# Crocodoctopus/zkstark

Measured on AMD Instinct MI355X. Metric: field-elements/s through LDE+Merkle+FRI (full STARK-101 prover), higher is better.
Workload: dtype u32 (mod 3*2^30+1) + SHA-256

## Files before the change

### zkstark_amd/csrc/host_sha.cpp

```cpp
#include "host_sha.hpp"

#include <atomic>

#if !defined(__HIP_DEVICE_COMPILE__)
#include <immintrin.h>
#include <stdlib.h>
#include <string.h>

namespace zk {
namespace {

#define ZK_SHA_TARGET __attribute__((target("sha,sse4.1,ssse3")))

alignas(16) const uint32_t K[64] = {
    0x428a2f98u, 0x71374491u, 0xb5c0fbcfu, 0xe9b5dba5u, 0x3956c25bu, 0x59f111f1u, 0x923f82a4u, 0xab1c5ed5u,
    0xd807aa98u, 0x12835b01u, 0x243185beu, 0x550c7dc3u, 0x72be5d74u, 0x80deb1feu, 0x9bdc06a7u, 0xc19bf174u,
    0xe49b69c1u, 0xefbe4786u, 0x0fc19dc6u, 0x240ca1ccu, 0x2de92c6fu, 0x4a7484aau, 0x5cb0a9dcu, 0x76f988dau,
    0x983e5152u, 0xa831c66du, 0xb00327c8u, 0xbf597fc7u, 0xc6e00bf3u, 0xd5a79147u, 0x06ca6351u, 0x14292967u,
    0x27b70a85u, 0x2e1b2138u, 0x4d2c6dfcu, 0x53380d13u, 0x650a7354u, 0x766a0abbu, 0x81c2c92eu, 0x92722c85u,
    0xa2bfe8a1u, 0xa81a664bu, 0xc24b8b70u, 0xc76c51a3u, 0xd192e819u, 0xd6990624u, 0xf40e3585u, 0x106aa070u,
    0x19a4c116u, 0x1e376c08u, 0x2748774cu, 0x34b0bcb5u, 0x391c0cb3u, 0x4ed8aa4au, 0x5b9cca4fu, 0x682e6ff3u,
    0x748f82eeu, 0x78a5636fu, 0x84c87814u, 0x8cc70208u, 0x90befffau, 0xa4506cebu, 0xbef9a3f7u, 0xc67178f2u};
const uint32_t IV[8] = {0x6a09e667u, 0xbb67ae85u, 0x3c6ef372u, 0xa54ff53au, 0x510e527fu, 0x9b05688cu, 0x1f83d9abu, 0x5be0cd19u};

alignas(16) uint32_t PADKW[64];
bool g_cpu_has_sha = false, g_cpu_has_x16 = false;
std::atomic<bool> g_have_sha{false}, g_have_x16{false};
std::atomic<bool> g_want_x16{true};

inline uint32_t rotr(uint32_t x, int n) { return (x >> n) | (x << (32 - n)); }

struct Init {
    Init() {
        __builtin_cpu_init();
        g_cpu_has_sha = __builtin_cpu_supports("sha") && __builtin_cpu_supports("sse4.1") && __builtin_cpu_supports("ssse3");
        g_cpu_has_x16 = g_cpu_has_sha && __builtin_cpu_supports("avx512f");
        g_have_sha = g_cpu_has_sha;
        g_have_x16 = g_cpu_has_x16;
        uint32_t w[64] = {0x80000000u};
        w[15] = 512u;
        for (int t = 16; t < 64; ++t) {
            uint32_t s0 = rotr(w[t - 15], 7) ^ rotr(w[t - 15], 18) ^ (w[t - 15] >> 3);
            uint32_t s1 = rotr(w[t - 2], 17) ^ rotr(w[t - 2], 19) ^ (w[t - 2] >> 10);
            w[t] = w[t - 16] + s0 + w[t - 7] + s1;
        }
        for (int t = 0; t < 64; ++t) PADKW[t] = K[t] + w[t];
    }
} g_init;

ZK_SHA_TARGET inline void load_state(const uint32_t st[8], __m128i& s0, __m128i& s1) {
    __m128i t = _mm_loadu_si128((const __m128i*)st);
    s1 = _mm_loadu_si128((const __m128i*)(st + 4));
    t = _mm_shuffle_epi32(t, 0xB1);
    s1 = _mm_shuffle_epi32(s1, 0x1B);
    s0 = _mm_alignr_epi8(t, s1, 8);
    s1 = _mm_blend_epi16(s1, t, 0xF0);
}
ZK_SHA_TARGET inline void store_state(uint32_t st[8], __m128i s0, __m128i s1) {
    __m128i t = _mm_shuffle_epi32(s0, 0x1B);
    s1 = _mm_shuffle_epi32(s1, 0xB1);
    s0 = _mm_blend_epi16(t, s1, 0xF0);
    s1 = _mm_alignr_epi8(s1, t, 8);
    _mm_storeu_si128((__m128i*)st, s0);
    _mm_storeu_si128((__m128i*)(st + 4), s1);
}

ZK_SHA_TARGET inline void rounds_msg(__m128i& s0, __m128i& s1, __m128i m[4]) {
    const __m128i a0 = s0, a1 = s1;
#pragma GCC unroll 16
    for (int g = 0; g < 16; ++g) {
        __m128i cur = m[g & 3];
        __m128i msg = _mm_add_epi32(cur, _mm_load_si128((const __m128i*)(K + 4 * g)));
        s1 = _mm_sha256rnds2_epu32(s1, s0, msg);
        if (g >= 3 && g <= 14) {
            __m128i t = _mm_alignr_epi8(cur, m[(g + 3) & 3], 4);
            m[(g + 1) & 3] = _mm_sha256msg2_epu32(_mm_add_epi32(m[(g + 1) & 3], t), cur);
        }
        msg = _mm_shuffle_epi32(msg, 0x0E);
        s0 = _mm_sha256rnds2_epu32(s0, s1, msg);
        if (g >= 1 && g <= 12) m[(g + 3) & 3] = _mm_sha256msg1_epu32(m[(g + 3) & 3], cur);
    }
    s0 = _mm_add_epi32(s0, a0);
    s1 = _mm_add_epi32(s1, a1);
}
ZK_SHA_TARGET inline void rounds_pad64(__m128i& s0, __m128i& s1) {
    const __m128i a0 = s0, a1 = s1;
#pragma GCC unroll 16
    for (int g = 0; g < 16; ++g) {
        __m128i msg = _mm_load_si128((const __m128i*)(PADKW + 4 * g));
        s1 = _mm_sha256rnds2_epu32(s1, s0, msg);
        msg = _mm_shuffle_epi32(msg, 0x0E);
        s0 = _mm_sha256rnds2_epu32(s0, s1, msg);
    }
    s0 = _mm_add_epi32(s0, a0);
    s1 = _mm_add_epi32(s1, a1);
}

ZK_SHA_TARGET void inner_ni(const uint32_t* l, const uint32_t* r, uint32_t* out) {
    __m128i s0, s1, m[4];
    load_state(IV, s0, s1);
    m[0] = _mm_loadu_si128((const __m128i*)l);
    m[1] = _mm_loadu_si128((const __m128i*)(l + 4));
    m[2] = _mm_loadu_si128((const __m128i*)r);
    m[3] = _mm_loadu_si128((const __m128i*)(r + 4));
    rounds_msg(s0, s1, m);
    rounds_pad64(s0, s1);
    store_state(out, s0, s1);
}
ZK_SHA_TARGET void inner_ni_x2(const uint32_t* in, uint32_t* out) {
    __m128i s0, s1, u0, u1, m[4], n[4];
    load_state(IV, s0, s1);
    u0 = s0; u1 = s1;
    const __m128i a0 = s0, a1 = s1;
    for (int i = 0; i < 4; ++i) {
        m[i] = _mm_loadu_si128((const __m128i*)(in + 4 * i));
        n[i] = _mm_loadu_si128((const __m128i*)(in + 16 + 4 * i));
    }
#pragma GCC unroll 16
    for (int g = 0; g < 16; ++g) {
        const __m128i k = _mm_load_si128((const __m128i*)(K + 4 * g));
        __m128i cm = m[g & 3], cn = n[g & 3];
        __m128i xm = _mm_add_epi32(cm, k), xn = _mm_add_epi32(cn, k);
        s1 = _mm_sha256rnds2_epu32(s1, s0, xm);
        u1 = _mm_sha256rnds2_epu32(u1, u0, xn);
        if (g >= 3 && g <= 14) {
            __m128i tm = _mm_alignr_epi8(cm, m[(g + 3) & 3], 4), tn = _mm_alignr_epi8(cn, n[(g + 3) & 3], 4);
            m[(g + 1) & 3] = _mm_sha256msg2_epu32(_mm_add_epi32(m[(g + 1) & 3], tm), cm);
            n[(g + 1) & 3] = _mm_sha256msg2_epu32(_mm_add_epi32(n[(g + 1) & 3], tn), cn);
        }
        xm = _mm_shuffle_epi32(xm, 0x0E);
        xn = _mm_shuffle_epi32(xn, 0x0E);
        s0 = _mm_sha256rnds2_epu32(s0, s1, xm);
        u0 = _mm_sha256rnds2_epu32(u0, u1, xn);
        if (g >= 1 && g <= 12) {
            m[(g + 3) & 3] = _mm_sha256msg1_epu32(m[(g + 3) & 3], cm);
            n[(g + 3) & 3] = _mm_sha256msg1_epu32(n[(g + 3) & 3], cn);
        }
    }
    s0 = _mm_add_epi32(s0, a0); s1 = _mm_add_epi32(s1, a1);
    u0 = _mm_add_epi32(u0, a0); u1 = _mm_add_epi32(u1, a1);
    const __m128i b0 = s0, b1 = s1, c0 = u0, c1 = u1;
#pragma GCC unroll 16
    for (int g = 0; g < 16; ++g) {
        __m128i msg = _mm_load_si128((const __m128i*)(PADKW + 4 * g));
        s1 = _mm_sha256rnds2_epu32(s1, s0, msg);
        u1 = _mm_sha256rnds2_epu32(u1, u0, msg);
        msg = _mm_shuffle_epi32(msg, 0x0E);
        s0 = _mm_sha256rnds2_epu32(s0, s1, msg);
        u0 = _mm_sha256rnds2_epu32(u0, u1, msg);
    }
    s0 = _mm_add_epi32(s0, b0); s1 = _mm_add_epi32(s1, b1);
    u0 = _mm_add_epi32(u0, c0); u1 = _mm_add_epi32(u1, c1);
    store_state(out, s0, s1);
    store_state(out + 8, u0, u1);
}
ZK_SHA_TARGET void compress_ni(uint32_t* st, const uint32_t* blk) {
    __m128i s0, s1, m[4];
    load_state(st, s0, s1);
    for (int i = 0; i < 4; ++i) m[i] = _mm_loadu_si128((const __m128i*)(blk + 4 * i));
    rounds_msg(s0, s1, m);
    store_state(st, s0, s1);
}
ZK_SHA_TARGET void blocks_ni(uint32_t* st, const uint8_t* data, size_t blocks) {
    const __m128i be = _mm_set_epi64x(0x0c0d0e0f08090a0bLL, 0x0405060700010203LL);
    __m128i s0, s1, m[4];
    load_state(st, s0, s1);
    for (; blocks; --blocks, data += 64) {
        for (int i = 0; i < 4; ++i) m[i] = _mm_shuffle_epi8(_mm_loadu_si128((const __m128i*)(data + 16 * i)), be);
        rounds_msg(s0, s1, m);
    }
    store_state(st, s0, s1);
}
ZK_SHA_TARGET void leaf_ni(uint32_t v, uint32_t* out) {
    __m128i s0, s1, m[4];
    load_state(IV, s0, s1);
    m[0] = _mm_set_epi32(0, 0, (int)0x80000000u, (int)v);
    m[1] = _mm_setzero_si128();
    m[2] = _mm_setzero_si128();
    m[3] = _mm_set_epi32(32, 0, 0, 0);
    rounds_msg(s0, s1, m);
    store_state(out, s0, s1);
}
#define ZK_X16_TARGET __attribute__((target("avx512f")))
#define ZK_ROR(x, n) _mm512_ror_epi32((x), (n))
#define ZK_XOR3(a, b, c) _mm512_ternarylogic_epi32((a), (b), (c), 0x96)

ZK_X16_TARGET inline void transpose16(__m512i r[16]) {
    __m512i t[16], u[16];
    for (int i = 0; i < 8; ++i) {
        t[2 * i] = _mm512_unpacklo_epi32(r[2 * i], r[2 * i + 1]);
        t[2 * i + 1] = _mm512_unpackhi_epi32(r[2 * i], r[2 * i + 1]);
    }
    for (int i = 0; i < 16; i += 4) {
        u[i] = _mm512_unpacklo_epi64(t[i], t[i + 2]);
        u[i + 1] = _mm512_unpackhi_epi64(t[i], t[i + 2]);
        u[i + 2] = _mm512_unpacklo_epi64(t[i + 1], t[i + 3]);
        u[i + 3] = _mm512_unpackhi_epi64(t[i + 1], t[i + 3]);
    }
    for (int k = 0; k < 4; ++k) {
        t[k] = _mm512_shuffle_i32x4(u[k], u[4 + k], 0x88);
        t[4 + k] = _mm512_shuffle_i32x4(u[k], u[4 + k], 0xdd);
        t[8 + k] = _mm512_shuffle_i32x4(u[8 + k], u[12 + k], 0x88);
        t[12 + k] = _mm512_shuffle_i32x4(u[8 + k], u[12 + k], 0xdd);
    }
    for (int k = 0; k < 4; ++k) {
        r[k] = _mm512_shuffle_i32x4(t[k], t[8 + k], 0x88);
        r[8 + k] = _mm512_shuffle_i32x4(t[k], t[8 + k], 0xdd);
        r[4 + k] = _mm512_shuffle_i32x4(t[4 + k], t[12 + k], 0x88);
        r[12 + k] = _mm512_shuffle_i32x4(t[4 + k], t[12 + k], 0xdd);
    }
}

template <bool MSG>
ZK_X16_TARGET inline void rounds_x16(__m512i st[8], __m512i w[16]) {
    __m512i a = st[0], b = st[1], c = st[2], d = st[3], e = st[4], f = st[5], g = st[6], h = st[7];
#pragma GCC unroll 64
    for (int t = 0; t < 64; ++t) {
        __m512i wk;
        if (MSG) {
            if (t >= 16) {
                const __m512i w15 = w[(t + 1) & 15], w2 = w[(t + 14) & 15];
                const __m512i s0 = ZK_XOR3(ZK_ROR(w15, 7), ZK_ROR(w15, 18), _mm512_srli_epi32(w15, 3));
                const __m512i s1 = ZK_XOR3(ZK_ROR(w2, 17), ZK_ROR(w2, 19), _mm512_srli_epi32(w2, 10));
                w[t & 15] = _mm512_add_epi32(_mm512_add_epi32(w[t & 15], s0), _mm512_add_epi32(w[(t + 9) & 15], s1));
            }
            wk = _mm512_add_epi32(w[t & 15], _mm512_set1_epi32((int)K[t]));
        } else {
            wk = _mm512_set1_epi32((int)PADKW[t]);
        }
        const __m512i S1 = ZK_XOR3(ZK_ROR(e, 6), ZK_ROR(e, 11), ZK_ROR(e, 25));
        const __m512i t1 = _mm512_add_epi32(_mm512_add_epi32(h, S1), _mm512_add_epi32(_mm512_ternarylogic_epi32(e, f, g, 0xCA), wk));
        const __m512i S0 = ZK_XOR3(ZK_ROR(a, 2), ZK_ROR(a, 13), ZK_ROR(a, 22));
        const __m512i t2 = _mm512_add_epi32(S0, _mm512_ternarylogic_epi32(a, b, c, 0xE8));
        h = g; g = f; f = e; e = _mm512_add_epi32(d, t1); d = c; c = b; b = a; a = _mm512_add_epi32(t1, t2);
    }
    st[0] = _mm512_add_epi32(st[0], a); st[1] = _mm512_add_epi32(st[1], b); st[2] = _mm512_add_epi32(st[2], c); st[3] = _mm512_add_epi32(st[3], d);
    st[4] = _mm512_add_epi32(st[4], e); st[5] = _mm512_add_epi32(st[5], f); st[6] = _mm512_add_epi32(st[6], g); st[7] = _mm512_add_epi32(st[7], h);
}
ZK_X16_TARGET inline void store_x16(const __m512i st[8], uint32_t* out) {
    __m512i r[16];
    for (int i = 0; i < 8; ++i) { r[i] = st[i]; r[8 + i] = _mm512_setzero_si512(); }
    transpose16(r);
    for (int n = 0; n < 16; ++n) _mm256_storeu_si256((__m256i*)(out + 8 * n), _mm512_castsi512_si256(r[n]));
}
ZK_X16_TARGET void inner_x16(const uint32_t* in, uint32_t* out) {
    __m512i w[16], st[8];
    for (int n = 0; n < 16; ++n) w[n] = _mm512_loadu_si512((const void*)(in + 16 * n));
    transpose16(w);
    for (int i = 0; i < 8; ++i) st[i] = _mm512_set1_epi32((int)IV[i]);
    rounds_x16<true>(st, w);
    rounds_x16<false>(st, w);
    store_x16(st, out);
}
ZK_X16_TARGET void leaves_x16(const uint32_t* vals, uint32_t* out) {
    __m512i w[16], st[8];
    w[0] = _mm512_loadu_si512((const void*)vals);
    w[1] = _mm512_set1_epi32((int)0x80000000u);
    for (int i = 2; i < 15; ++i) w[i] = _mm512_setzero_si512();
    w[15] = _mm512_set1_epi32(32);
    for (int i = 0; i < 8; ++i) st[i] = _mm512_set1_epi32((int)IV[i]);
    rounds_x16<true>(st, w);
    store_x16(st, out);
}

void inner_run(const uint32_t* child, uint32_t* out, size_t cnt) {
    size_t i = 0;
    if (g_have_x16)
        for (; i + 16 <= cnt; i += 16) inner_x16(child + 16 * i, out + 8 * i);
    for (; i + 2 <= cnt; i += 2) inner_ni_x2(child + 16 * i, out + 8 * i);
    for (; i < cnt; ++i) inner_ni(child + 16 * i, child + 16 * i + 8, out + 8 * i);
}

ZK_SHA_TARGET void reduce_ni(uint32_t* nodes, uint32_t depth) {
    for (uint32_t d = depth; d-- > 0;) {
        const size_t base = ((size_t)1 << d) - 1, child = ((size_t)2 << d) - 1, cnt = (size_t)1 << d;
        inner_run(nodes + 8 * child, nodes + 8 * base, cnt);
    }
}

ZK_SHA_TARGET void reduce_sub_ni(uint32_t* nodes, uint32_t depth, uint32_t top, size_t sub) {
    for (uint32_t d = depth; d-- > top;) {
        const size_t cnt = (size_t)1 << (d - top);
        const size_t base = ((size_t)1 << d) - 1 + sub * cnt, child = ((size_t)2 << d) - 1 + 2 * sub * cnt;
        inner_run(nodes + 8 * child, nodes + 8 * base, cnt);
    }
}

void compress_generic(uint32_t st[8], const uint32_t blk[16]) {
    uint32_t w[64];
    memcpy(w, blk, 64);
    for (int t = 16; t < 64; ++t) {
        uint32_t s0 = rotr(w[t - 15], 7) ^ rotr(w[t - 15], 18) ^ (w[t - 15] >> 3);
        uint32_t s1 = rotr(w[t - 2], 17) ^ rotr(w[t - 2], 19) ^ (w[t - 2] >> 10);
        w[t] = w[t - 16] + s0 + w[t - 7] + s1;
    }
    uint32_t a = st[0], b = st[1], c = st[2], d = st[3], e = st[4], f = st[5], g = st[6], h = st[7];
    for (int t = 0; t < 64; ++t) {
        uint32_t t1 = h + (rotr(e, 6) ^ rotr(e, 11) ^ rotr(e, 25)) + ((e & f) ^ (~e & g)) + K[t] + w[t];
        uint32_t t2 = (rotr(a, 2) ^ rotr(a, 13) ^ rotr(a, 22)) + ((a & b) ^ (a & c) ^ (b & c));
        h = g; g = f; f = e; e = d + t1; d = c; c = b; b = a; a = t1 + t2;
    }
    st[0] += a; st[1] += b; st[2] += c; st[3] += d; st[4] += e; st[5] += f; st[6] += g; st[7] += h;
}

}

bool host_sha_available() { return g_have_sha; }
void host_sha_use_extensions(bool on) {
    g_have_sha = on && g_cpu_has_sha;
    g_have_x16 = on && g_cpu_has_x16 && g_want_x16.load(std::memory_order_relaxed);
}
bool host_sha_wide_available() { return g_have_x16; }
void host_sha_use_wide(bool on) {
    g_want_x16 = on;
    g_have_x16 = on && g_have_sha.load(std::memory_order_relaxed) && g_cpu_has_x16;
}

void host_sha_compress(uint32_t state[8], const uint32_t block[16]) {
    if (g_have_sha) compress_ni(state, block);
    else compress_generic(state, block);
}

void host_sha_blocks(uint32_t state[8], const uint8_t* data, size_t blocks) {
    if (g_have_sha) { blocks_ni(state, data, blocks); return; }
    for (; blocks; --blocks, data += 64) {
        uint32_t w[16];
        for (int i = 0; i < 16; ++i)
            w[i] = ((uint32_t)data[4 * i] << 24) | ((uint32_t)data[4 * i + 1] << 16) | ((uint32_t)data[4 * i + 2] << 8) | data[4 * i + 3];
        compress_generic(state, w);
    }
}

void host_sha_leaf(uint32_t v, uint32_t out[8]) {
    if (g_have_sha) { leaf_ni(v, out); return; }
    uint32_t blk[16] = {v, 0x80000000u, 0, 0, 0, 0, 0, 0, 0, 0, 0, 0, 0, 0, 0, 32u};
    uint32_t st[8];
    memcpy(st, IV, 32);
    compress_generic(st, blk);
    memcpy(out, st, 32);
}

void host_sha_leaves(const uint32_t* vals, size_t n, uint32_t* out) {
    size_t i = 0;
    if (g_have_x16)
        for (; i + 16 <= n; i += 16) leaves_x16(vals + i, out + 8 * i);
    for (; i < n; ++i) host_sha_leaf(vals[i], out + 8 * i);
}

void host_sha_inner(const uint32_t left[8], const uint32_t right[8], uint32_t out[8]) {
    if (g_have_sha) { inner_ni(left, right, out); return; }
    uint32_t blk[16], st[8];
    memcpy(blk, left, 32);
    memcpy(blk + 8, right, 32);
    memcpy(st, IV, 32);
    compress_generic(st, blk);
    uint32_t pad[16] = {0x80000000u, 0, 0, 0, 0, 0, 0, 0, 0, 0, 0, 0, 0, 0, 0, 512u};
    compress_generic(st, pad);
    memcpy(out, st, 32);
}

void host_sha_inner_run(const uint32_t* children, uint32_t* out, size_t cnt) {
    if (g_have_sha) { inner_run(children, out, cnt); return; }
    for (size_t i = 0; i < cnt; ++i) host_sha_inner(children + 16 * i, children + 16 * i + 8, out + 8 * i);
}

void host_sha_reduce_sub(uint32_t* nodes, uint32_t depth, uint32_t top, size_t sub) {
    if (g_have_sha) { reduce_sub_ni(nodes, depth, top, sub); return; }
    for (uint32_t d = depth; d-- > top;) {
        const size_t cnt = (size_t)1 << (d - top);
        const size_t base = ((size_t)1 << d) - 1 + sub * cnt, child = ((size_t)2 << d) - 1 + 2 * sub * cnt;
        for (size_t i = 0; i < cnt; ++i)
            host_sha_inner(nodes + 8 * (child + 2 * i), nodes + 8 * (child + 2 * i + 1), nodes + 8 * (base + i));
    }
}

void host_sha_reduce(uint32_t* nodes, uint32_t depth) {
    if (g_have_sha) { reduce_ni(nodes, depth); return; }
    for (uint32_t d = depth; d-- > 0;) {
        const size_t base = ((size_t)1 << d) - 1, child = ((size_t)2 << d) - 1, cnt = (size_t)1 << d;
        for (size_t i = 0; i < cnt; ++i)
            host_sha_inner(nodes + 8 * (child + 2 * i), nodes + 8 * (child + 2 * i + 1), nodes + 8 * (base + i));
    }
}

}
#endif
```

### zkstark_amd/csrc/host_sha.hpp

```cpp
#pragma once
#include <stddef.h>
#include <stdint.h>

namespace zk {

bool host_sha_available();
void host_sha_use_extensions(bool on);
bool host_sha_wide_available();
void host_sha_use_wide(bool on);
void host_sha_compress(uint32_t state[8], const uint32_t block[16]);
void host_sha_blocks(uint32_t state[8], const uint8_t* data, size_t blocks);
void host_sha_leaf(uint32_t v, uint32_t out[8]);
void host_sha_leaves(const uint32_t* vals, size_t n, uint32_t* out);
void host_sha_inner(const uint32_t left[8], const uint32_t right[8], uint32_t out[8]);
void host_sha_inner_run(const uint32_t* children, uint32_t* out, size_t cnt);
void host_sha_reduce(uint32_t* nodes, uint32_t depth);
void host_sha_reduce_sub(uint32_t* nodes, uint32_t depth, uint32_t top, size_t sub);

}
```

### zkstark_amd/csrc/zkstark.hip

```cpp
#include <hip/hip_runtime.h>

#include <algorithm>
#include <chrono>
#include <cstdarg>
#include <cstdio>
#include <cstdlib>
#include <cstring>
#include <atomic>
#include <condition_variable>
#include <functional>
#include <mutex>
#include <new>
#include <thread>
#include <string>
#include <vector>

#include "../../include/zkstark_amd.h"
#include "field.hpp"
#include "kernels.hpp"
#include "sha256.hpp"
#include "transcript.hpp"
#include "host_sha.hpp"
#include "internal.hpp"
#include "pool.hpp"

using namespace zk;
using namespace zk::impl;

struct zk_ctx {
    int device = 0;
    uint32_t log_n = 0, log_b = 0, L = 0;
    size_t n = 0, N = 0, B = 0;
    uint32_t R = 0;
    hipStream_t stream = nullptr;
    zk_dom* dom = nullptr;
    uint32_t* d_trace = nullptr;
    uint32_t* d_coef = nullptr;
    uint32_t* d_layers = nullptr;
    std::vector<size_t> layer_off, layer_len;
    uint32_t* d_trees = nullptr;
    std::vector<size_t> tree_off;
    uint64_t* d_gather_off = nullptr;
    uint32_t* d_gather_out = nullptr;
    uint64_t* h_gather_off = nullptr;
    uint32_t* h_gather_out = nullptr;
    uint64_t* dm_gather_off = nullptr;
    uint32_t* dm_gather_out = nullptr;
    const uint32_t* host_nodes[40] = {};
    size_t host_node_cnt[40] = {};
    const uint32_t* host_vals[40] = {};
    std::vector<const uint32_t*> fetch_vals, fetch_nodes;
    std::vector<uint32_t> fetch_vdev;
    std::vector<uint64_t> fetch_ditems;
    std::vector<uint8_t> commit_buf;
    bool pending_top = false;
    uint32_t pending_tree = 0;
    size_t open_nv = 0, open_ndg = 0, open_vi = 0;
    bool open_pending = false;
    uint32_t* h_small = nullptr;
    uint32_t* h_mailbox = nullptr;
    uint32_t* d_mailbox = nullptr;
    uint32_t* d_counter = nullptr;
    bool counters_dirty = false;
    uint32_t mail_seq = 0;
    uint32_t tree_seq[40] = {};
    bool early = false, early_ok = false, gate_pending = false;
    uint32_t* h_gate = nullptr;
    uint32_t* d_gate = nullptr;
    uint32_t* h_dyn = nullptr;
    uint32_t* d_dyn = nullptr;
    uint32_t gate_seq = 0;
    uint32_t host_top = 0, host_tail = 0;
    Pool* pool = nullptr;
    uint32_t* h_stage = nullptr;
    uint32_t* d_stage = nullptr;
    size_t stage_words = 0, stage_used = 0;
    ScatterSeg* h_segs = nullptr;
    ScatterSeg* d_segs = nullptr;
    uint32_t n_segs = 0;
    double seg_words = 0;
    std::vector<uint32_t> tail_vals;
    uint32_t tail_log = 0;
    bool tail_have = false;
    double t_wait = 0, t_host_hash = 0, t_launch = 0;
    bool tail = false;
    uint32_t hinv_host = 0;
    ProofFormat fmt;
    Grinder* grinder = nullptr;
    uint64_t skipped_layers = 0, skipped_trees = 0;
    uint8_t tree_steps[40] = {};
    uint32_t* d_final = nullptr;
    std::vector<uint32_t> final_poly;
    int hash = 0;
    uint32_t cap_now = 0;
    uint8_t tree_cap[40] = {};
    std::vector<uint8_t> cap_digests[40];
    bool checks = false;
    uint32_t* d_check = nullptr;
    DevTable ones;
    size_t gather_cap = 0;
    size_t device_bytes = 0;
    double setup_ms = 0;
    bool have_trace = false, have_lde = false;
    uint32_t first = 0, last = 0;
    zk_transcript_info info{};
    Profiler prof;
    zk_kernel_stat kstat[K_COUNT] = {};
};

namespace {

template <typename T>
int dmalloc(zk_ctx* c, T** p, size_t bytes) {
    hipError_t e = hipMalloc((void**)p, bytes ? bytes : 4);
    if (e != hipSuccess) return fail(ZK_ERR_NOMEM, "hipMalloc(%zu) failed: %s", bytes, hipGetErrorString(e));
    c->device_bytes += bytes;
    return ZK_OK;
}

size_t layer_size(const zk_ctx* c, uint32_t layer) { return layer == 0 ? c->N : (c->N >> (layer - 1)); }
uint32_t layer_log(const zk_ctx* c, uint32_t layer) { return layer == 0 ? c->L : c->L - (layer - 1); }
uint32_t tree_log(const zk_ctx* c, uint32_t tree) { return layer_log(c, tree) - c->tree_steps[tree]; }
size_t tree_leaves(const zk_ctx* c, uint32_t tree) { return (size_t)1 << tree_log(c, tree); }

Profiler* prof_of(zk_ctx* c) { return c->prof.mask ? &c->prof : nullptr; }

void collect_kernel_stats(zk_ctx* c) {
    for (auto& r : c->prof.recs) {
        float ms = 0;
        (void)hipEventSynchronize(r.b);
        (void)hipEventElapsedTime(&ms, r.a, r.b);
        c->kstat[r.cls].launches += 1;
        c->kstat[r.cls].ms += ms;
        c->kstat[r.cls].bytes += r.bytes;
        c->kstat[r.cls].ops += r.ops;
        c->prof.pool.push_back(r.a);
        c->prof.pool.push_back(r.b);
    }
    c->prof.recs.clear();
}

int do_lde(zk_ctx* c) {
    int rc = dom_lde(c->dom, c->d_trace, c->d_coef, c->d_layers + c->layer_off[0], c->stream, prof_of(c));
    if (!rc) c->have_lde = true;
    return rc;
}

#ifndef ZK_HOST_SUB_LOG
#define ZK_HOST_SUB_LOG 8
#endif
static_assert(ZK_HOST_SUB_LOG >= 4 && ZK_HOST_SUB_LOG <= (int)kMaxHostLog, "host sub-tree size");
constexpr uint32_t host_sub_log() { return ZK_HOST_SUB_LOG; }
uint32_t top_of(const zk_ctx* c, uint32_t tree) {
    if (c->hash != 0 || !c->host_top) return 0;
    const uint32_t lg = tree_log(c, tree);
    return lg > c->host_top ? c->host_top : lg - 1;
}
uint32_t cap_of(const zk_ctx* c, uint32_t tree) { return c->cap_now ? cap_eff(c->cap_now, tree_log(c, tree)) : 0; }
uint32_t hand_of(const zk_ctx* c, uint32_t tree) {
    const uint32_t h = top_of(c, tree), ce = cap_of(c, tree);
    return h > ce ? h : ce;
}
MailArgs mail_of(zk_ctx* c, uint32_t tree, bool host, bool feed_tail = true, uint32_t steps = 0) {
    MailArgs m;
    c->tree_steps[tree] = (uint8_t)steps;
    if (c->counters_dirty) {
        (void)hipMemsetAsync(c->d_counter, 0, 64, c->stream);
        c->counters_dirty = false;
    }
    m.mailbox = c->d_mailbox;
    m.seq = ++c->mail_seq;
    c->tree_seq[tree] = m.seq;
    m.counter = c->d_counter;
    const uint32_t host_levels = host ? top_of(c, tree) : 0;
    c->tree_cap[tree] = (uint8_t)(host ? cap_of(c, tree) : 0);
    m.top = host ? hand_of(c, tree) : 0;
    if (feed_tail && c->fmt.fold == 1 && !c->fmt.coset && !c->fmt.stop && host_levels && c->host_tail && tree >= 1 && layer_log(c, tree) == c->host_tail + 1) {
        m.dump_src = c->d_layers + c->layer_off[tree];
        m.dump_log = c->host_tail + 1;
        m.vals_off = (uint32_t)kMailValsOff;
        c->tail_log = m.dump_log;
        c->tail_have = true;
    }
    return m;
}

int do_merkle(zk_ctx* c, uint32_t layer, bool host = false, bool feed_tail = true, uint32_t steps = 0) {
    HIPCHK(launch_merkle_build_coset(c->d_layers + c->layer_off[layer], layer_log(c, layer), steps, c->d_trees + c->tree_off[layer], c->stream,
                                     prof_of(c), mail_of(c, layer, host, feed_tail, steps), c->hash));
    return ZK_OK;
}

int do_compose_commit(zk_ctx* c, const uint32_t alpha_raw[3]) {
    ComposeArgs a;
    int rc = compose_args(c->dom, c->d_layers + c->layer_off[0], c->d_layers + c->layer_off[1], c->first, c->last, alpha_raw, a);
    if (rc) return rc;
    HIPCHK(launch_compose_merkle(a, c->d_trees + c->tree_off[1], c->stream, prof_of(c), mail_of(c, 1, true), c->hash));
    return ZK_OK;
}
int do_fold_commit(zk_ctx* c, uint32_t round, uint32_t beta_raw) {
    FoldArgs a;
    int rc = fold_args(c->dom, c->d_layers + c->layer_off[1 + round], c->d_layers + c->layer_off[2 + round], c->L - round, round, beta_raw, a);
    if (rc) return rc;
    HIPCHK(launch_fold_merkle(a, c->d_trees + c->tree_off[2 + round], c->stream, prof_of(c), mail_of(c, 2 + round, true), c->hash));
    return ZK_OK;
}

int wait_mail(zk_ctx* c, uint32_t seq) {
    double t0 = now_us();
    int rc = wait_flag(c->h_mailbox, seq, c->stream);
    c->t_wait += now_us() - t0;
    if (rc) c->counters_dirty = true;
    return rc;
}

int read_root(zk_ctx* c, uint32_t tree, uint8_t out[32]) {
    int rc = wait_mail(c, c->tree_seq[tree]);
    if (rc) return rc;
    digest_words_to_bytes(c->h_mailbox + kMailDigests, out);
    return ZK_OK;
}

uint32_t* stage_alloc(zk_ctx* c, size_t words) {
    if (c->stage_used + words > c->stage_words) return nullptr;
    uint32_t* p = c->h_stage + c->stage_used;
    c->stage_used += (words + 7) & ~(size_t)7;
    return p;
}
int stage_seg(zk_ctx* c, const uint32_t* src, size_t dst, size_t words, uint32_t kind) {
    if (c->n_segs >= 4 * 34) return fail(ZK_ERR_STATE, "scatter segment table full");
    c->h_segs[c->n_segs++] = ScatterSeg{(uint64_t)(src - c->h_stage), (uint64_t)dst, (uint32_t)words, kind};
    c->seg_words += (double)words;
    return ZK_OK;
}

int read_commit_cap(zk_ctx* c, uint32_t tree, uint32_t H, uint32_t ce, uint8_t root[32]) {
    const size_t cnt = (size_t)1 << H, first = ((size_t)1 << ce) - 1, ncap = (size_t)1 << ce;
    uint32_t* nodes = stage_alloc(c, (2 * cnt - 1) * 8);
    if (!nodes) return fail(ZK_ERR_STATE, "host staging buffer exhausted");
    int rc = wait_mail(c, c->tree_seq[tree]);
    if (rc) return rc;
    double t0 = now_us();
    memcpy(nodes + 8 * (cnt - 1), c->h_mailbox + kMailDigests, cnt * 32);
    if (H > ce) {
        if (c->pool) c->pool->run(ncap, 1, [&](size_t sub) { host_sha_reduce_sub(nodes, H, ce, sub); });
        else for (size_t sub = 0; sub < ncap; ++sub) host_sha_reduce_sub(nodes, H, ce, sub);
    }
    std::vector<uint8_t>& cd = c->cap_digests[tree];
    cd.resize(32 * ncap);
    for (size_t i = 0; i < ncap; ++i) digest_words_to_bytes(nodes + 8 * (first + i), cd.data() + 32 * i);
    memset(root, 0, 32);
    c->t_host_hash += now_us() - t0;
    if (c->tail_have && c->tail_log == layer_log(c, tree) && tree >= 1) {
        c->tail_vals.assign(c->h_mailbox + kMailValsOff, c->h_mailbox + kMailValsOff + ((size_t)1 << c->tail_log));
    }
    c->host_nodes[tree] = nodes;
    c->host_node_cnt[tree] = 2 * cnt - 1;
    return H > ce ? stage_seg(c, nodes + 8 * first, c->tree_off[tree] + 8 * first, (cnt - 1 - first) * 8, 0) : (int)ZK_OK;
}

int read_commit(zk_ctx* c, uint32_t tree, uint8_t root[32]) {
    const uint32_t H = hand_of(c, tree), ce = cap_of(c, tree);
    if (!H) return read_root(c, tree, root);
    if (ce) return read_commit_cap(c, tree, H, ce, root);
    const size_t cnt = (size_t)1 << H;
    uint32_t* nodes = stage_alloc(c, (2 * cnt - 1) * 8);
    if (!nodes) return fail(ZK_ERR_STATE, "host staging buffer exhausted");
    int rc = wait_mail(c, c->tree_seq[tree]);
    if (rc) return rc;
    double t0 = now_us();
    memcpy(nodes + 8 * (cnt - 1), c->h_mailbox + kMailDigests, cnt * 32);
    const uint32_t sub_log = host_sub_log();
    if (H > sub_log && c->pool) {
        const uint32_t top = H - sub_log;
        c->pool->run((size_t)1 << top, 1, [&](size_t sub) { host_sha_reduce_sub(nodes, H, top, sub); });
        host_sha_reduce(nodes, top);
    } else {
        host_sha_reduce(nodes, H);
    }
    digest_words_to_bytes(nodes, root);
    c->t_host_hash += now_us() - t0;
    if (c->tail_have && c->tail_log == layer_log(c, tree) && tree >= 1) {
        c->tail_vals.assign(c->h_mailbox + kMailValsOff, c->h_mailbox + kMailValsOff + ((size_t)1 << c->tail_log));
    }
    c->host_nodes[tree] = nodes;
    c->host_node_cnt[tree] = 2 * cnt - 1;
    return stage_seg(c, nodes, c->tree_off[tree], (cnt - 1) * 8, 0);
}

int host_fold_commit(zk_ctx* c, uint32_t round, uint32_t beta_raw, uint8_t root[32]) {
    const uint32_t log_out = c->L - round - 1;
    const size_t half = (size_t)1 << log_out;
    const double t_begin = now_us();
    uint32_t* vals = stage_alloc(c, half);
    uint32_t* nodes = stage_alloc(c, (2 * half - 1) * 8);
    if (!vals || !nodes) return fail(ZK_ERR_STATE, "host staging buffer exhausted");
    const zk_dom* d = c->dom;
    const uint32_t cc_m = to_mont(mulmod(beta_raw % P, d->fold_k[round]));
    const uint32_t step_m = to_mont(powmod(c->hinv_host, (uint64_t)1 << round));
    const uint32_t* in = c->tail_vals.data();
    uint32_t xinv_m = to_mont(1);
    for (size_t i = 0; i < half; ++i) {
        uint32_t u = in[i], v = in[i + half];
        vals[i] = add(mont_mul(add(u, v), d->inv2_mont), mont_mul(mont_mul(sub(u, v), xinv_m), cc_m));
        xinv_m = mont_mul(xinv_m, step_m);
    }
    host_sha_leaves(vals, half, nodes + 8 * (half - 1));
    host_sha_reduce(nodes, log_out);
    digest_words_to_bytes(nodes, root);
    c->tail_vals.assign(vals, vals + half);
    c->tail_log = log_out;
    c->t_host_hash += now_us() - t_begin;
    c->tree_steps[2 + round] = 0;
    c->tree_cap[2 + round] = (uint8_t)cap_of(c, 2 + round);
    if (const uint32_t ce = c->tree_cap[2 + round]) {
        std::vector<uint8_t>& cd = c->cap_digests[2 + round];
        cd.resize((size_t)32 << ce);
        for (size_t i = 0; i < ((size_t)1 << ce); ++i) digest_words_to_bytes(nodes + 8 * (((size_t)1 << ce) - 1 + i), cd.data() + 32 * i);
        memset(root, 0, 32);
    }
    c->host_vals[2 + round] = vals;
    c->host_nodes[2 + round] = nodes;
    c->host_node_cnt[2 + round] = 2 * half - 1;
    int rc = stage_seg(c, vals, c->layer_off[2 + round], half, 1);
    if (!rc) rc = stage_seg(c, nodes, c->tree_off[2 + round], (2 * half - 1) * 8, 0);
    return rc;
}

int fri_round_commit(zk_ctx* c, uint32_t round, uint32_t beta_raw, uint8_t root[32]) {
    if (c->tail_have && c->tail_log == c->L - round && c->L - round - 1 <= c->host_tail) return host_fold_commit(c, round, beta_raw, root);
    int rc = do_fold_commit(c, round, beta_raw);
    return rc ? rc : read_commit(c, 2 + round, root);
}
bool round_on_host(const zk_ctx* c, uint32_t round) {
    return c->hash == 0 && c->host_top && c->host_tail && c->L >= c->host_tail + 1 && c->L - round <= c->host_tail + 1;
}
bool can_gate(const zk_ctx* c, uint32_t round) { return c->fmt.fold == 1 && !c->fmt.coset && !c->fmt.stop && c->early && c->early_ok && !c->checks && round < c->R && !round_on_host(c, round); }
int enqueue_gated_fold(zk_ctx* c, uint32_t round) {
    FoldArgs a;
    int rc = fold_args(c->dom, c->d_layers + c->layer_off[1 + round], c->d_layers + c->layer_off[2 + round], c->L - round, round, 0u, a);
    if (rc) return rc;
    ++c->gate_seq;
    a.dyn = c->d_dyn + 16 * (c->gate_seq & 1u);
    HIPCHK(hipStreamWaitValue32(c->stream, c->d_gate, c->gate_seq, hipStreamWaitValueEq, 0xFFFFFFFFu));
    c->gate_pending = true;
    HIPCHK(launch_fold_merkle(a, c->d_trees + c->tree_off[2 + round], c->stream, prof_of(c), mail_of(c, 2 + round, true), c->hash));
    return ZK_OK;
}
void release_gate(zk_ctx* c, uint32_t c_mont) {
    c->h_dyn[16 * (c->gate_seq & 1u)] = c_mont;
    __atomic_store_n(c->h_gate, c->gate_seq, __ATOMIC_RELEASE);
    c->gate_pending = false;
}
void release_gated_fold(zk_ctx* c, uint32_t round, uint32_t beta_raw) {
    release_gate(c, to_mont(mulmod(beta_raw % P, c->dom->fold_k[round])));
}
struct GateGuard {
    zk_ctx* c;
    ~GateGuard() { if (c->gate_pending) release_gate(c, 0u); }
};

struct CapScope {
    zk_ctx* c;
    explicit CapScope(zk_ctx* ctx) : c(ctx) { c->cap_now = c->tail ? 0 : c->fmt.cap; }
    ~CapScope() { c->cap_now = 0; }
};

void begin_proof(zk_ctx* c) {
    c->stage_used = 0; c->n_segs = 0; c->seg_words = 0; c->tail_log = 0; c->tail_have = false;
    c->t_wait = c->t_host_hash = c->t_launch = 0;
    memset(c->host_nodes, 0, sizeof c->host_nodes);
    memset(c->host_node_cnt, 0, sizeof c->host_node_cnt);
    memset(c->host_vals, 0, sizeof c->host_vals);
}
int flush_host_parts(zk_ctx* c) {
    HIPCHK(launch_scatter(c->d_stage, c->d_segs, c->n_segs, c->seg_words, c->d_trees, c->d_layers, c->stream, prof_of(c)));
    c->n_segs = 0;
    c->pending_top = false;
    return ZK_OK;
}
int settle_pending(zk_ctx* c) { return c->pending_top ? flush_host_parts(c) : (int)ZK_OK; }
int last_layer_value(zk_ctx* c, uint32_t* out) {
    const uint32_t* v;
    if (c->tail_have && c->tail_log == c->log_b) v = c->tail_vals.data();
    else {
        HIPCHK(hipMemcpyAsync(c->h_small, c->d_layers + c->layer_off[1 + c->R], c->B * 4, hipMemcpyDeviceToHost, c->stream));
        HIPCHK(hipStreamSynchronize(c->stream));
        v = c->h_small;
    }
    for (size_t i = 1; i < c->B; ++i)
        if (v[i] != v[0]) return fail(ZK_ERR_CHECK, "last FRI layer is not constant (prover.rs:238): trace does not satisfy the constraints");
    *out = v[0];
    return ZK_OK;
}

int final_alloc(zk_ctx* c) {
    return c->d_final ? (int)ZK_OK : dmalloc(c, &c->d_final, (((size_t)1 << kFinalPolyMaxLog) + 1) * 4);
}
int final_poly_value(zk_ctx* c) {
    const uint32_t Rp = c->fmt.rounds();
    const size_t cnt = (size_t)1 << c->fmt.stop;
    int rc = final_alloc(c);
    if (rc) return rc;
    if ((rc = dom_final_poly(c->dom, c->d_layers + c->layer_off[1 + Rp], c->d_final, c->L - Rp, Rp, (uint32_t)cnt, c->stream, prof_of(c)))) return rc;
    HIPCHK(hipMemcpyAsync(c->h_small, c->d_final, (cnt + 1) * 4, hipMemcpyDeviceToHost, c->stream));
    HIPCHK(hipStreamSynchronize(c->stream));
    if (c->h_small[0])
        return fail(ZK_ERR_CHECK, "final FRI layer has degree >= 2^%u: trace does not satisfy the constraints (%u non-zero coefficients above; cf. prover.rs:238)", c->fmt.stop, c->h_small[0]);
    c->final_poly.assign(c->h_small + 1, c->h_small + 1 + cnt);
    return ZK_OK;
}

int do_compose(zk_ctx* c, const uint32_t alpha_raw[3]) {
    return dom_compose(c->dom, c->d_layers + c->layer_off[0], c->d_layers + c->layer_off[1], c->first, c->last,
                       alpha_raw, c->stream, prof_of(c));
}

int do_fold(zk_ctx* c, uint32_t round, uint32_t beta_raw) {
    return dom_fold(c->dom, c->d_layers + c->layer_off[1 + round], c->d_layers + c->layer_off[2 + round],
                    c->L - round, round, beta_raw, c->stream, prof_of(c));
}


int checks_alloc(zk_ctx* c) {
    if (c->d_check) return ZK_OK;
    int rc = dmalloc(c, &c->d_check, (c->N + 2) * 4);
    if (rc) return rc;
    return build_table(1, c->log_n, &c->ones);
}
int check_interpolant(zk_ctx* c) {
    const zk_dom* d = c->dom;
    CoefPrepArgs pa{};
    pa.log_n = d->log_n; pa.log_b = d->log_b;
    pa.tw = d->H.view(); pa.wtab = c->ones.view(); pa.ninv_mont = d->ninv_mont;
    pa.nd = d->plan.nd;
    for (uint32_t t = 0; t < d->plan.nd; ++t) pa.dig_bits[t] = d->plan.bits[t];
    HIPCHK(launch_coef_prepare(c->d_coef, c->d_check, pa, c->stream));
    int rc = run_dit(c->d_check, d->log_n, d->plan, d->H.view(), d->L, c->stream);
    if (rc) return rc;
    std::vector<uint32_t> got(c->n), want(c->n);
    HIPCHK(hipMemcpyAsync(got.data(), c->d_check, c->n * 4, hipMemcpyDeviceToHost, c->stream));
    HIPCHK(hipMemcpyAsync(want.data(), c->d_trace, c->n * 4, hipMemcpyDeviceToHost, c->stream));
    HIPCHK(hipStreamSynchronize(c->stream));
    for (size_t i = 0; i + 1 < c->n; ++i)
        if (got[i] != want[i])
            return fail(ZK_ERR_CHECK, "self-check prover.rs:64-66 failed: f(g^%zu) = %u, trace value %u", i, got[i], want[i]);
    return ZK_OK;
}
int check_degree(zk_ctx* c, uint32_t layer, uint32_t want_deg, const char* cite) {
    const uint32_t lg = layer_log(c, layer);
    const size_t m = (size_t)1 << lg;
    const uint32_t* src = c->d_layers + c->layer_off[layer];
    if (lg <= 10) {
        std::vector<uint32_t> v(m);
        if (c->tail_have && c->tail_log == lg && layer >= 2) v.assign(c->tail_vals.begin(), c->tail_vals.begin() + m);
        else {
            HIPCHK(hipMemcpyAsync(v.data(), src, m * 4, hipMemcpyDeviceToHost, c->stream));
            HIPCHK(hipStreamSynchronize(c->stream));
        }
        const uint32_t winv = invmod(root_of_unity(lg));
        for (size_t k = m; k-- > want_deg; ) {
            uint32_t acc = 0, step = powmod(winv, k), x = 1;
            for (size_t i = 0; i < m; ++i) { acc = add(acc, mulmod(v[i], x)); x = mulmod(x, step); }
            if (k > want_deg && acc != 0)
                return fail(ZK_ERR_CHECK, "self-check %s failed: layer %u has a non-zero coefficient of degree %zu > %u", cite, layer, k, want_deg);
            if (k == want_deg && acc == 0)
                return fail(ZK_ERR_CHECK, "self-check %s failed: layer %u has degree below %u", cite, layer, want_deg);
        }
        return ZK_OK;
    }
    const Plan pl = make_plan(lg);
    int rc = run_dif(src, c->d_check, lg, pl, c->dom->Hinv.view(), c->dom->L, 0, c->stream);
    if (rc) return rc;
    uint32_t* res = c->d_check + c->N;
    HIPCHK(hipMemsetAsync(res, 0, 8, c->stream));
    HIPCHK(launch_degree_check(c->d_check, lg, pl.nd, pl.bits, want_deg + 1, res, c->stream));
    uint32_t h[2];
    HIPCHK(hipMemcpyAsync(h, res, 8, hipMemcpyDeviceToHost, c->stream));
    HIPCHK(hipStreamSynchronize(c->stream));
    if (h[0]) return fail(ZK_ERR_CHECK, "self-check %s failed: layer %u has %u non-zero coefficients of degree > %u (a division left a remainder)", cite, layer, h[0], want_deg);
    if (!h[1]) return fail(ZK_ERR_CHECK, "self-check %s failed: layer %u has degree below %u", cite, layer, want_deg);
    return ZK_OK;
}

void open_begin(zk_ctx* c, size_t nvals) {
    c->fetch_vals.assign(nvals, nullptr); c->fetch_vdev.assign(nvals, 0); c->fetch_nodes.clear(); c->fetch_ditems.clear();
    c->open_nv = c->open_ndg = c->open_vi = 0;
}
void open_val(zk_ctx* c, uint32_t layer, size_t x) {
    if (c->host_vals[layer]) c->fetch_vals[c->open_vi++] = c->host_vals[layer] + x;
    else { c->fetch_vdev[c->open_vi++] = (uint32_t)c->open_nv; c->h_gather_off[c->open_nv++] = (uint64_t)c->layer_off[layer] + x; }
}
void open_path(zk_ctx* c, uint32_t tree, size_t m, size_t leaf) {
    const size_t stop_at = ((size_t)2 << c->tree_cap[tree]) - 2;
    for (size_t i = leaf + m - 1; i > stop_at; i = (i - 1) >> 1) {
        const size_t nd = (i & 1) ? i + 1 : i - 1;
        if (nd < c->host_node_cnt[tree]) c->fetch_nodes.push_back(c->host_nodes[tree] + 8 * nd);
        else { c->fetch_nodes.push_back(c->h_gather_out + 8 * c->open_ndg); ++c->open_ndg; c->fetch_ditems.push_back((uint64_t)c->tree_off[tree] + (uint64_t)nd * 8); }
    }
}
int open_launch(zk_ctx* c) {
    const size_t nv = c->open_nv, ndg = c->open_ndg;
    if (nv + ndg > c->gather_cap) return fail(ZK_ERR_STATE, "gather capacity exceeded");
    if (ndg) memcpy(c->h_gather_off + nv, c->fetch_ditems.data(), ndg * 8);
    for (size_t i = 0; i < c->fetch_vals.size(); ++i)
        if (!c->fetch_vals[i]) c->fetch_vals[i] = c->h_gather_out + 8 * ndg + c->fetch_vdev[i];
    c->open_pending = nv + ndg != 0;
    if (c->open_pending)
        HIPCHK(launch_fetch(c->d_layers, c->d_trees, c->dm_gather_off, (uint32_t)nv, (uint32_t)ndg, c->dm_gather_out, c->d_mailbox,
                            ++c->mail_seq, c->d_counter, c->stream, prof_of(c)));
    return ZK_OK;
}
int open_wait(zk_ctx* c) {
    if (!c->open_pending) return ZK_OK;
    c->open_pending = false;
    return wait_mail(c, c->mail_seq);
}

void commit_tree(zk_ctx* c, Channel& ch, uint32_t tree, const uint8_t root[32]) {
    if (c->tree_cap[tree]) { ch.commit_bytes(c->cap_digests[tree].data(), c->cap_digests[tree].size()); return; }
    ch.commit_hash(root);
    memcpy(c->info.roots[tree], root, 32);
}

int prove_fold_rounds(zk_ctx* c, Channel& ch) {
    const ProofFormat& f = c->fmt;
    const uint32_t R = f.rounds(), G = f.groups();
    uint8_t root[32];
    int rc;
    for (uint32_t j = 0; j < G; ++j) {
        const uint32_t r0 = f.round0(j), steps = f.steps(j), id = f.tree_id(j + 1);
        const uint32_t beta = c->info.beta_raw[r0] = ch.get_u32();
        if ((rc = dom_fold_multi(c->dom, c->d_layers + c->layer_off[1 + r0], c->d_layers + c->layer_off[id], c->L - r0, r0, steps, beta,
                                 c->stream, prof_of(c)))) return rc;
        const bool stopped = f.stop && j + 1 == G;
        if (!stopped && ((rc = do_merkle(c, id, true, false, f.slots_log(j + 1))) || (rc = read_commit(c, id, root)))) return rc;
        const size_t deg = c->n >> (r0 + steps);
        if (c->checks && (rc = check_degree(c, id, (uint32_t)deg - (deg ? 1 : 0), "prover.rs:228-251 (FRI layer degree)"))) return rc;
        if (!stopped) commit_tree(c, ch, id, root);
        for (uint32_t l = 2 + r0; l < id; ++l) { c->skipped_layers |= (uint64_t)1 << l; c->skipped_trees |= (uint64_t)1 << l; }
    }
    if (f.stop) {
        c->skipped_trees |= (uint64_t)1 << (1 + R);
        for (uint32_t l = 2 + R; l <= c->R + 1; ++l) { c->skipped_layers |= (uint64_t)1 << l; c->skipped_trees |= (uint64_t)1 << l; }
    }
    return ZK_OK;
}

struct HostLaps {
    const bool on;
    std::chrono::steady_clock::time_point t0 = std::chrono::steady_clock::now();
    void operator()(const char* what) {
        if (!on) return;
        auto t = std::chrono::steady_clock::now();
        fprintf(stderr, "[zk timing] %-28s %8.1f us\n", what, std::chrono::duration<double, std::micro>(t - t0).count());
        t0 = t;
    }
};

int prove_finish(zk_ctx* c, Channel& ch, HostLaps& lap) {
    const ProofFormat& f = c->fmt;
    const uint32_t Q = f.q;
    const size_t B = c->B, N = c->N;
    int rc;
    if (c->fmt.stop) {
        if ((rc = final_poly_value(c))) return rc;
        c->info.free_term = c->final_poly[0];
        std::vector<uint8_t>& cb = c->commit_buf;
        cb.resize(4 * c->final_poly.size());
        for (size_t k = 0; k < c->final_poly.size(); ++k)
            for (int i = 0; i < 4; ++i) cb[4 * k + i] = (uint8_t)(c->final_poly[k] >> (8 * i));
        ch.commit_bytes(cb.data(), cb.size());
    } else {
        uint32_t free_term = 0;
        if ((rc = last_layer_value(c, &free_term))) return rc;
        c->info.free_term = free_term;
        ch.commit_u32(free_term);
        c->final_poly.assign(1, free_term);
    }
    if (c->fmt.grind) {
        uint64_t w = 0;
        if ((rc = grind_channel(c->grinder, ch, c->fmt.grind, &w))) return rc;
        c->info.grind_bits = c->fmt.grind;
        c->info.grind_nonce = w;
        lap("grind");
    }
    uint32_t qraws[64];
    for (uint32_t k = 0; k < Q; ++k) qraws[k] = ch.get_u32();
    c->info.query_raw = qraws[0];

    size_t per_query = 0;
    f.for_each_tuple([&](size_t s, size_t, bool) { per_query += s; });
    open_begin(c, (size_t)Q * per_query);
    for (uint32_t k = 0; k < Q; ++k)
        f.for_each_opening((size_t)qraws[k] % (N - 2 * B), [&](uint32_t layer, uint32_t log_leaves, size_t leaf, uint32_t slots_log) {
            for (size_t u = 0; u < ((size_t)1 << slots_log); ++u) open_val(c, layer, leaf + (u << log_leaves));
            open_path(c, layer, (size_t)1 << log_leaves, leaf);
        });
    if ((rc = open_launch(c))) return rc;
    if ((rc = flush_host_parts(c))) return rc;
    lap("free term + fetch enqueue");
    if ((rc = open_wait(c))) return rc;
    lap("fetch wait");
    const uint32_t* const* vsrc = c->fetch_vals.data();
    const uint32_t* const* dsrc = c->fetch_nodes.data();
    std::vector<uint8_t>& buf = c->commit_buf;
    buf.resize(Channel::group_bytes((size_t)1 << f.steps(0), f.L(), false));
    auto tuple = [&](size_t s, size_t plen, bool one_leaf) {
        ch.commit_group(buf.data(), s, plen, [&](size_t t) { return *vsrc[t]; },
                        [&](size_t i, uint8_t* out) { digest_words_to_bytes(dsrc[i], out); }, one_leaf);
        vsrc += s; dsrc += (one_leaf ? 1 : s) * plen;
    };
    for (uint32_t q = 0; q < Q; ++q) f.for_each_tuple(tuple);
    lap("decommit host hashing");
    return ZK_OK;
}

int prove_resident(zk_ctx* c, Channel& ch) {
    if (!c->have_trace) return fail(ZK_ERR_STATE, "zk_prove_resident: no trace uploaded");
    static const bool timing = getenv("ZK_HOST_TIMING") != nullptr;
    HostLaps lap{timing};
    const uint32_t R = c->R;
    ch.data.reserve(ch.data.size() + c->fmt.data_len());
    CapScope cap_scope{c};
    c->skipped_layers = c->skipped_trees = 0;
    uint8_t root[32];
    int rc;
    memset(&c->info, 0, sizeof c->info);
    c->info.public_last = c->last;
    c->pending_top = false;
    begin_proof(c);
    GateGuard gate_guard{c};
    if ((rc = do_lde(c))) return rc;
    if (c->checks && ((rc = checks_alloc(c)) || (rc = check_interpolant(c)))) return rc;
    if ((rc = do_merkle(c, 0, true))) return rc;
    if ((rc = read_commit(c, 0, root))) return rc;
    commit_tree(c, ch, 0, root);
    uint32_t alpha[3];
    for (int i = 0; i < 3; ++i) alpha[i] = c->info.alpha_raw[i] = ch.get_u32();
    if (c->fmt.coset) {
        if ((rc = do_compose(c, alpha)) || (rc = do_merkle(c, 1, true, false, c->fmt.steps(0)))) return rc;
    } else if ((rc = do_compose_commit(c, alpha))) return rc;
    if (can_gate(c, 0) && (rc = enqueue_gated_fold(c, 0))) return rc;
    if ((rc = read_commit(c, 1, root))) return rc;
    if (c->checks && (rc = check_degree(c, 1, (uint32_t)c->n - 1, "prover.rs:148-159/:169 (exact divisions, deg cp = n - 1)"))) return rc;
    commit_tree(c, ch, 1, root);
    if (c->fmt.fold > 1 || c->fmt.coset || c->fmt.stop) {
        if ((rc = prove_fold_rounds(c, ch))) return rc;
    } else for (uint32_t r = 0; r < R; ++r) {
        uint32_t beta = c->info.beta_raw[r] = ch.get_u32();
        if (c->gate_pending) {
            release_gated_fold(c, r, beta);
            if (can_gate(c, r + 1) && (rc = enqueue_gated_fold(c, r + 1))) return rc;
            if ((rc = read_commit(c, 2 + r, root))) return rc;
        } else if (c->tail_have && c->tail_log == c->L - r && c->L - r - 1 <= c->host_tail) {
            if ((rc = host_fold_commit(c, r, beta, root))) return rc;
        } else {
            if ((rc = do_fold_commit(c, r, beta))) return rc;
            if (can_gate(c, r + 1) && (rc = enqueue_gated_fold(c, r + 1))) return rc;
            if ((rc = read_commit(c, 2 + r, root))) return rc;
        }
        if (c->checks && (rc = check_degree(c, 2 + r, (uint32_t)(c->n >> (r + 1)) - ((c->n >> (r + 1)) ? 1 : 0), "prover.rs:228-251 (FRI layer degree)"))) return rc;
        commit_tree(c, ch, 2 + r, root);
    }
    lap("lde .. last root");
    if (timing) fprintf(stderr, "[zk timing]   of which: waiting for the device %.1f us, host hashing (tops + tail) %.1f us\n", c->t_wait, c->t_host_hash);
    return prove_finish(c, ch, lap);
}

}

namespace zk {
namespace impl {
int tail_open_begin(zk_ctx* c, size_t x) {
    if (!c || !c->tail) return fail(ZK_ERR_INVALID, "tail_open_begin: not a tail context");
    HIPCHK(hipSetDevice(c->device));
    open_begin(c, 2 * (size_t)c->R);
    for (uint32_t i = 0; i < c->R; ++i) {
        const size_t len = c->N >> i, xi = x % len, nx = (xi + len / 2) % len;
        open_val(c, 1 + i, xi); open_path(c, 1 + i, len, xi);
        open_val(c, 1 + i, nx); open_path(c, 1 + i, len, nx);
    }
    return open_launch(c);
}
int tail_open_end(zk_ctx* c, uint32_t* vals_out, uint8_t* paths_out) {
    int rc = open_wait(c);
    if (rc) return rc;
    for (size_t i = 0; i < c->fetch_vals.size(); ++i) vals_out[i] = *c->fetch_vals[i];
    for (size_t i = 0; i < c->fetch_nodes.size(); ++i) digest_words_to_bytes(c->fetch_nodes[i], paths_out + 32 * i);
    return ZK_OK;
}
int merkle_nodes_to_host(int device, hipStream_t s, const uint32_t* d_heap, size_t first, size_t count, uint8_t* out) {
    if (!count) return ZK_OK;
    HIPCHK(hipSetDevice(device));
    HIPCHK(hipMemcpyAsync(out, d_heap + first * 8, count * 32, hipMemcpyDeviceToHost, s));
    HIPCHK(hipStreamSynchronize(s));
    for (size_t i = 0; i < count; ++i) {
        uint32_t w[8];
        memcpy(w, out + 32 * i, 32);
        digest_words_to_bytes(w, out + 32 * i);
    }
    return ZK_OK;
}
}
}

extern "C" {

const char* zk_last_error(void) { return last_error(); }
int zk_host_hash_mode(void) { return host_sha_wide_available() ? 2 : host_sha_available() ? 1 : 0; }
int zk_host_set_hash_mode(int mode) {
    if (mode < 0 || mode > 2) return fail(ZK_ERR_INVALID, "zk_host_set_hash_mode: mode %d out of range (0 portable, 1 SHA extensions, 2 + AVX-512)", mode);
    host_sha_use_extensions(mode >= 1);
    host_sha_use_wide(mode >= 2);
    return ZK_OK;
}

uint32_t zk_field_add(uint32_t a, uint32_t b) { return add(a % P, b % P); }
uint32_t zk_field_sub(uint32_t a, uint32_t b) { return sub(a % P, b % P); }
uint32_t zk_field_mul(uint32_t a, uint32_t b) { return mulmod(a % P, b % P); }
uint32_t zk_field_neg(uint32_t a) { return neg(a % P); }
uint32_t zk_field_inv(uint32_t a) { return invmod(a % P); }
uint32_t zk_field_pow(uint32_t a, uint32_t e) { return powmod(a, e); }
uint32_t zk_field_from_u32(uint32_t v) { return v % P; }
uint32_t zk_field_from_i32(int32_t v) {
    if (v < 0) return neg(uint32_t(-int64_t(v)) % P);
    return uint32_t(v) % P;
}
uint32_t zk_field_div(uint32_t a, uint32_t b) {
    if (b % P == 0) { fail(ZK_ERR_INVALID, "zk_field_div: division by zero (field.rs:165-177 panics)"); return 0; }
    return mulmod(a % P, invmod(b % P));
}
uint32_t zk_field_rem(uint32_t a, uint32_t rhs) {
    if (rhs == 0) { fail(ZK_ERR_INVALID, "zk_field_rem: remainder by zero (field.rs:89-94 panics)"); return 0; }
    return (a % P) % rhs;
}
uint32_t zk_field_generator(void) {
    static const uint32_t g = [] {
        uint32_t factors[32], nf = 0, p = P - 1;
        for (uint32_t it = 2; p != 1; ++it) {
            if (p % it == 0) factors[nf++] = it;
            while (p % it == 0) p /= it;
        }
        for (uint32_t x = 2; x < P; ++x) {
            bool primitive = true;
            for (uint32_t i = 0; i < nf && primitive; ++i) primitive = powmod(x, (P - 1) / factors[i]) != 1;
            if (primitive) return x;
        }
        return 0u;
    }();
    return g;
}
uint32_t zk_field_order(uint32_t a) {
    a %= P;
    if (a == 0) return 0;
    uint32_t ord = P - 1;
    if (powmod(a, ord / 3) == 1) ord /= 3;
    while (ord % 2 == 0 && powmod(a, ord / 2) == 1) ord /= 2;
    return ord;
}
uint32_t zk_field_root_of_unity(uint32_t log_order) { return log_order > 30 ? 0 : root_of_unity(log_order); }

static int ctx_make(int device, uint32_t log_n, uint32_t log_b, uint32_t shift, bool tail, zk_ctx** out);
static int ctx_team(zk_ctx* c) {
    const uint32_t sub_log = host_sub_log();
    const unsigned want = c->host_top > sub_log ? (1u << (c->host_top - sub_log)) - 1u : 0u;
    if (c->pool && c->pool->workers() == want) return ZK_OK;
    delete c->pool;
    c->pool = nullptr;
    if (!want) return ZK_OK;
    const double spin_us = 5000.0;
    c->pool = new (std::nothrow) Pool(want, spin_us);
    return c->pool ? (int)ZK_OK : fail(ZK_ERR_NOMEM, "out of host memory");
}

int zk_ctx_create(int device, uint32_t log_n, uint32_t log_b, zk_ctx** out) {
    if (!out) return fail(ZK_ERR_INVALID, "zk_ctx_create: out is null");
    *out = nullptr;
    if (int rc = check_proof_size("zk_ctx_create", log_n, log_b)) return rc;
    return ctx_make(device, log_n, log_b, GEN_W, false, out);
}

static int ctx_make(int device, uint32_t log_n, uint32_t log_b, uint32_t shift, bool tail, zk_ctx** out) {
    auto t0 = std::chrono::steady_clock::now();
    HIPCHK(hipSetDevice(device));
    zk_ctx* c = new (std::nothrow) zk_ctx();
    if (!c) return fail(ZK_ERR_NOMEM, "out of host memory");
    c->device = device;
    c->log_n = log_n; c->log_b = log_b; c->L = log_n + log_b;
    c->fmt.log_n = log_n; c->fmt.log_b = log_b;
    c->n = (size_t)1 << log_n; c->B = (size_t)1 << log_b; c->N = c->n << log_b;
    c->R = log_n;
    int rc = ZK_OK;
    auto bail = [&](int code) { zk_ctx_destroy(c); return code; };
#define HIPCHK_C(expr)                                                                        \
    do {                                                                                      \
        hipError_t _e = (expr);                                                               \
        if (_e != hipSuccess) {                                                               \
            zk_ctx_destroy(c);                                                                \
            return fail(ZK_ERR_HIP, "%s failed: %s (%s:%d)", #expr, hipGetErrorString(_e), __FILE__, __LINE__); \
        }                                                                                     \
    } while (0)
    HIPCHK_C(hipStreamCreateWithFlags(&c->stream, hipStreamNonBlocking));
    if ((rc = dom_make(device, log_n, log_b, shift, tail, c->stream, &c->dom))) return bail(rc);
    c->tail = tail;
    c->hinv_host = invmod(c->dom->h);
    c->device_bytes += c->dom->device_bytes;
    size_t off = 0;
    for (uint32_t l = 0; l <= c->R + 1; ++l) {
        c->layer_off.push_back(off);
        c->layer_len.push_back(layer_size(c, l));
        off += layer_size(c, l);
    }
    size_t layer_words = off;
    off = 0;
    for (uint32_t l = 0; l <= c->R + 1; ++l) {
        c->tree_off.push_back(off);
        off += (2 * layer_size(c, l) - 1) * 8;
    }
    size_t tree_words = off;
    if ((rc = dmalloc(c, &c->d_trace, c->n * 4))) return bail(rc);
    if ((rc = dmalloc(c, &c->d_coef, 2 * c->n * 4))) return bail(rc);
    if ((rc = dmalloc(c, &c->d_layers, layer_words * 4))) return bail(rc);
    if ((rc = dmalloc(c, &c->d_trees, tree_words * 4))) return bail(rc);
    c->gather_cap = (size_t)kMaxQueries * (4 + 2 * c->R) * (c->L + 1) + 64;
    if ((rc = dmalloc(c, &c->d_gather_off, c->gather_cap * 8))) return bail(rc);
    if ((rc = dmalloc(c, &c->d_gather_out, c->gather_cap * 32))) return bail(rc);
    HIPCHK_C(hipHostMalloc((void**)&c->h_gather_off, c->gather_cap * 8, hipHostMallocMapped | hipHostMallocCoherent));
    HIPCHK_C(hipHostMalloc((void**)&c->h_gather_out, c->gather_cap * 32, hipHostMallocMapped | hipHostMallocCoherent));
    HIPCHK_C(hipHostGetDevicePointer((void**)&c->dm_gather_off, c->h_gather_off, 0));
    HIPCHK_C(hipHostGetDevicePointer((void**)&c->dm_gather_out, c->h_gather_out, 0));
    HIPCHK_C(hipHostMalloc((void**)&c->h_small, 4096));
    const size_t mail_bytes = kMailWords * 4;
    if ((rc = dmalloc(c, &c->d_counter, 64))) return bail(rc);
    HIPCHK_C(hipMemsetAsync(c->d_counter, 0, 64, c->stream));
    HIPCHK_C(hipHostMalloc((void**)&c->h_mailbox, mail_bytes, hipHostMallocMapped | hipHostMallocCoherent));
    memset(c->h_mailbox, 0, mail_bytes);
    HIPCHK_C(hipHostGetDevicePointer((void**)&c->d_mailbox, c->h_mailbox, 0));
    HIPCHK_C(hipHostMalloc((void**)&c->h_gate, 64, hipHostMallocMapped | hipHostMallocCoherent));
    HIPCHK_C(hipHostMalloc((void**)&c->h_dyn, 2 * 16 * 4, hipHostMallocMapped | hipHostMallocCoherent));
    memset(c->h_gate, 0, 64);
    memset(c->h_dyn, 0, 2 * 16 * 4);
    HIPCHK_C(hipHostGetDevicePointer((void**)&c->d_gate, c->h_gate, 0));
    HIPCHK_C(hipHostGetDevicePointer((void**)&c->d_dyn, c->h_dyn, 0));
    {
        int can = 0;
        if (hipDeviceGetAttribute(&can, hipDeviceAttributeCanUseStreamWaitValue, device) != hipSuccess) { can = 0; (void)hipGetLastError(); }
        c->early_ok = can != 0 && !tail;
    }
    c->stage_words = (size_t)(c->R + 2) * ((size_t)16 << kMaxHostLog) + ((size_t)64 << kMaxHostLog);
    const size_t seg_bytes = 4 * 34 * sizeof(ScatterSeg);
    HIPCHK_C(hipHostMalloc((void**)&c->h_stage, c->stage_words * 4 + seg_bytes, hipHostMallocMapped | hipHostMallocCoherent));
    HIPCHK_C(hipHostGetDevicePointer((void**)&c->d_stage, c->h_stage, 0));
    c->h_segs = reinterpret_cast<ScatterSeg*>(c->h_stage + c->stage_words);
    c->d_segs = reinterpret_cast<ScatterSeg*>(c->d_stage + c->stage_words);
    if (host_sha_available()) {
        c->host_top = 8;
        c->host_tail = 9;
    }
    if (int prc = ctx_team(c)) { zk_ctx_destroy(c); return prc; }
#undef HIPCHK_C
    c->setup_ms = std::chrono::duration<double, std::milli>(std::chrono::steady_clock::now() - t0).count();
    *out = c;
    return ZK_OK;
}

#ifdef ZK_WG_TRACE
extern "C++" { namespace zk { void dump_wg_trace(); } }
#endif

int zk_ctx_destroy(zk_ctx* c) {
    if (!c) return ZK_OK;
    (void)hipSetDevice(c->device);
    if (c->stream) (void)hipStreamSynchronize(c->stream);
#ifdef ZK_WG_TRACE
    zk::dump_wg_trace();
#endif
    dom_free(c->dom);
    if (c->d_trace) (void)hipFree(c->d_trace);
    if (c->d_coef) (void)hipFree(c->d_coef);
    if (c->d_layers) (void)hipFree(c->d_layers);
    if (c->d_trees) (void)hipFree(c->d_trees);
    if (c->d_counter) (void)hipFree(c->d_counter);
    if (c->d_check) (void)hipFree(c->d_check);
    if (c->d_final) (void)hipFree(c->d_final);
    free_table(&c->ones);
    if (c->d_gather_off) (void)hipFree(c->d_gather_off);
    if (c->d_gather_out) (void)hipFree(c->d_gather_out);
    if (c->h_gather_off) (void)hipHostFree(c->h_gather_off);
    if (c->h_gather_out) (void)hipHostFree(c->h_gather_out);
    if (c->h_small) (void)hipHostFree(c->h_small);
    if (c->h_mailbox) (void)hipHostFree(c->h_mailbox);
    if (c->h_gate) (void)hipHostFree(c->h_gate);
    if (c->h_dyn) (void)hipHostFree(c->h_dyn);
    if (c->h_stage) (void)hipHostFree(c->h_stage);
    grinder_destroy(c->grinder);
    collect_kernel_stats(c);
    delete c->pool;
    for (hipEvent_t e : c->prof.pool) (void)hipEventDestroy(e);
    if (c->stream) (void)hipStreamDestroy(c->stream);
    delete c;
    return ZK_OK;
}

double zk_ctx_setup_ms(const zk_ctx* c) { return c ? c->setup_ms : 0.0; }
size_t zk_ctx_device_bytes(const zk_ctx* c) { return c ? c->device_bytes : 0; }
void* zk_ctx_stream(zk_ctx* c) {
    if (!c) return nullptr;
    if (c->pending_top && hipSetDevice(c->device) == hipSuccess) (void)settle_pending(c);
    return (void*)c->stream;
}
int zk_ctx_sync(zk_ctx* c) {
    if (!c) return fail(ZK_ERR_INVALID, "null context");
    HIPCHK(hipSetDevice(c->device));
    if (int rc = settle_pending(c)) return rc;
    HIPCHK(hipStreamSynchronize(c->stream));
    return ZK_OK;
}
int zk_ctx_set_early_launch(zk_ctx* c, int on) {
    if (!c) return fail(ZK_ERR_INVALID, "null context");
    c->early = on != 0;
    return ZK_OK;
}
int zk_ctx_get_early_launch(const zk_ctx* c) { return c && c->early && c->early_ok && c->fmt.fold == 1 && !c->fmt.coset && !c->fmt.stop ? 1 : 0; }
int zk_ctx_set_fold(zk_ctx* c, uint32_t fold_log) {
    if (!c) return fail(ZK_ERR_INVALID, "null context");
    if (c->tail) return fail(ZK_ERR_STATE, "zk_ctx_set_fold: FRI-tail context");
    if (fold_log < 1 || fold_log > kMaxFoldLog) return fail(ZK_ERR_INVALID, "zk_ctx_set_fold: need 1 <= fold_log <= %u (got %u)", kMaxFoldLog, fold_log);
    const ProofFormat widest{.log_n = c->log_n, .log_b = c->log_b, .fold = fold_log};
    size_t opened = 0;
    widest.for_each_tuple([&](size_t s, size_t, bool) { opened += s; });
    const size_t cap = (size_t)kMaxQueries * opened * (c->L + 1) + 64;
    if (cap > c->gather_cap) {
        HIPCHK(hipSetDevice(c->device));
        HIPCHK(hipStreamSynchronize(c->stream));
        uint64_t *d_off = nullptr, *h_off = nullptr, *dm_off = nullptr;
        uint32_t *d_out = nullptr, *h_out = nullptr, *dm_out = nullptr;
        hipError_t e = hipMalloc((void**)&d_off, cap * 8);
        if (e == hipSuccess) e = hipMalloc((void**)&d_out, cap * 32);
        if (e == hipSuccess) e = hipHostMalloc((void**)&h_off, cap * 8, hipHostMallocMapped | hipHostMallocCoherent);
        if (e == hipSuccess) e = hipHostMalloc((void**)&h_out, cap * 32, hipHostMallocMapped | hipHostMallocCoherent);
        if (e == hipSuccess) e = hipHostGetDevicePointer((void**)&dm_off, h_off, 0);
        if (e == hipSuccess) e = hipHostGetDevicePointer((void**)&dm_out, h_out, 0);
        if (e != hipSuccess) {
            if (d_off) (void)hipFree(d_off);
            if (d_out) (void)hipFree(d_out);
            if (h_off) (void)hipHostFree(h_off);
            if (h_out) (void)hipHostFree(h_out);
            return fail(ZK_ERR_NOMEM, "zk_ctx_set_fold: decommitment buffers: %s", hipGetErrorString(e));
        }
        (void)hipFree(c->d_gather_off); (void)hipFree(c->d_gather_out);
        (void)hipHostFree(c->h_gather_off); (void)hipHostFree(c->h_gather_out);
        c->d_gather_off = d_off; c->d_gather_out = d_out; c->h_gather_off = h_off; c->h_gather_out = h_out;
        c->dm_gather_off = dm_off; c->dm_gather_out = dm_out;
        c->device_bytes += (cap - c->gather_cap) * 40;
        c->gather_cap = cap;
    }
    c->fmt.fold = fold_log;
    return ZK_OK;
}
uint32_t zk_ctx_get_fold(const zk_ctx* c) { return c ? c->fmt.fold : 0; }
int zk_ctx_set_coset_leaves(zk_ctx* c, int on) {
    if (!c) return fail(ZK_ERR_INVALID, "null context");
    if (c->tail) return fail(ZK_ERR_STATE, "zk_ctx_set_coset_leaves: FRI-tail context");
    c->fmt.coset = on != 0;
    return ZK_OK;
}
int zk_ctx_get_coset_leaves(const zk_ctx* c) { return c && c->fmt.coset ? 1 : 0; }
int zk_ctx_set_fri_stop(zk_ctx* c, uint32_t stop_log) {
    if (!c) return fail(ZK_ERR_INVALID, "null context");
    if (c->tail) return fail(ZK_ERR_STATE, "zk_ctx_set_fri_stop: FRI-tail context");
    if (!stop_ok(c->log_n, c->log_b, stop_log))
        return fail(ZK_ERR_INVALID, "zk_ctx_set_fri_stop: need stop_log <= %u, stop_log <= log_n - 1 = %u and stop_log + log_blowup <= %u (got %u)",
                    kMaxStopLog, c->log_n - 1, kMaxStopLayerLog, stop_log);
    if (stop_log) {
        HIPCHK(hipSetDevice(c->device));
        if (int rc = final_alloc(c)) return rc;
    }
    c->fmt.stop = stop_log;
    return ZK_OK;
}
uint32_t zk_ctx_get_fri_stop(const zk_ctx* c) { return c ? c->fmt.stop : 0; }
int zk_ctx_final_poly(const zk_ctx* c, uint32_t* out, size_t cap, size_t* count) {
    if (!c || !count || (!out && cap)) return fail(ZK_ERR_INVALID, "zk_ctx_final_poly: null argument");
    if (c->final_poly.empty()) return fail(ZK_ERR_STATE, "zk_ctx_final_poly: no proof made yet");
    *count = c->final_poly.size();
    if (c->final_poly.size() > cap) return fail(ZK_ERR_BUFFER, "zk_ctx_final_poly: %zu coefficients, room for %zu", c->final_poly.size(), cap);
    memcpy(out, c->final_poly.data(), c->final_poly.size() * 4);
    return ZK_OK;
}
int zk_ctx_set_merkle_cap(zk_ctx* c, uint32_t cap_log) {
    if (!c) return fail(ZK_ERR_INVALID, "null context");
    if (c->tail) return fail(ZK_ERR_STATE, "zk_ctx_set_merkle_cap: FRI-tail context");
    if (cap_log > kMaxCapLog) return fail(ZK_ERR_INVALID, "zk_ctx_set_merkle_cap: need cap_log <= %u (got %u)", kMaxCapLog, cap_log);
    c->fmt.cap = cap_log;
    return ZK_OK;
}
uint32_t zk_ctx_get_merkle_cap(const zk_ctx* c) { return c ? c->fmt.cap : 0; }
uint32_t zk_ctx_merkle_cap_log(const zk_ctx* c, uint32_t tree) { return c && tree <= c->R + 1 ? c->tree_cap[tree] : 0; }
int zk_ctx_merkle_cap(const zk_ctx* c, uint32_t tree, uint8_t* out, size_t out_len) {
    if (!c || !out) return fail(ZK_ERR_INVALID, "zk_ctx_merkle_cap: null argument");
    if (tree > c->R + 1) return fail(ZK_ERR_INVALID, "zk_ctx_merkle_cap: tree %u out of range", tree);
    if (c->final_poly.empty()) return fail(ZK_ERR_STATE, "zk_ctx_merkle_cap: no proof made yet");
    if ((c->skipped_trees >> tree) & 1) return fail(ZK_ERR_STATE, "zk_ctx_merkle_cap: tree %u was not built by the last proof (fold_log %u, fri_stop %u)", tree, c->fmt.fold, c->fmt.stop);
    const uint32_t ce = c->tree_cap[tree];
    const uint8_t* src = ce ? c->cap_digests[tree].data() : c->info.roots[tree];
    if (((size_t)32 << ce) > out_len) return fail(ZK_ERR_BUFFER, "zk_ctx_merkle_cap: %zu bytes, room for %zu", (size_t)32 << ce, out_len);
    memcpy(out, src, (size_t)32 << ce);
    return ZK_OK;
}
int zk_ctx_set_queries(zk_ctx* c, uint32_t n_queries) {
    if (!c) return fail(ZK_ERR_INVALID, "null context");
    if (n_queries < 1 || n_queries > kMaxQueries) return fail(ZK_ERR_INVALID, "zk_ctx_set_queries: need 1 <= n_queries <= %u", kMaxQueries);
    c->fmt.q = n_queries;
    return ZK_OK;
}
int zk_ctx_set_grinding(zk_ctx* c, uint32_t grind_bits) {
    if (!c) return fail(ZK_ERR_INVALID, "null context");
    if (c->tail) return fail(ZK_ERR_STATE, "zk_ctx_set_grinding: FRI-tail context");
    if (grind_bits > kMaxGrindBits) return fail(ZK_ERR_INVALID, "zk_ctx_set_grinding: need grind_bits <= %u (got %u)", kMaxGrindBits, grind_bits);
    if (grind_bits > kGrindHostMaxBits && !c->grinder) {
        HIPCHK(hipSetDevice(c->device));
        if (int rc = grinder_create(c->device, c->stream, 1, &c->grinder)) return rc;
    }
    c->fmt.grind = grind_bits;
    return ZK_OK;
}

int zk_ctx_set_host_levels(zk_ctx* c, uint32_t top_log, uint32_t tail_log) {
    if (!c) return fail(ZK_ERR_INVALID, "null context");
    if (top_log > kMaxHostLog || tail_log > kMaxHostLog || (tail_log && !top_log))
        return fail(ZK_ERR_INVALID, "zk_ctx_set_host_levels: need top_log, tail_log <= %u, and top_log > 0 when tail_log > 0", kMaxHostLog);
    c->host_top = top_log;
    c->host_tail = tail_log;
    return ctx_team(c);
}
int zk_ctx_get_host_levels(const zk_ctx* c, uint32_t* top_log, uint32_t* tail_log) {
    if (!c || !top_log || !tail_log) return fail(ZK_ERR_INVALID, "zk_ctx_get_host_levels: null argument");
    *top_log = c->host_top;
    *tail_log = c->host_tail;
    return ZK_OK;
}
int zk_ctx_set_checks(zk_ctx* c, int on) {
    if (!c) return fail(ZK_ERR_INVALID, "null context");
    if (c->tail) return fail(ZK_ERR_STATE, "zk_ctx_set_checks: FRI-tail context");
    c->checks = on != 0;
    return ZK_OK;
}
static const char kNoBlake2s[] = "BLAKE2s (hash 2) is not built for this entry point yet";
int zk_ctx_set_hash(zk_ctx* c, int hash_kind) {
    if (!c) return fail(ZK_ERR_INVALID, "null context");
    if (hash_kind != ZK_HASH_SHA256 && hash_kind != ZK_HASH_FIELD && hash_kind != ZK_HASH_BLAKE2S)
        return fail(ZK_ERR_INVALID, "zk_ctx_set_hash: unknown hash %d", hash_kind);
    if (hash_kind == ZK_HASH_BLAKE2S && c->tail) return fail(ZK_ERR_INVALID, "zk_ctx_set_hash: %s", kNoBlake2s);
    c->hash = hash_kind;
    return ZK_OK;
}

int zk_ctx_set_profiling(zk_ctx* c, uint32_t class_mask) {
    if (!c) return fail(ZK_ERR_INVALID, "null context");
    c->prof.mask = class_mask & ((1u << K_COUNT) - 1u);
    return ZK_OK;
}

static int put_kernel_stats(zk_kernel_stat* out, size_t count, const zk_kernel_stat* src, const char* who) {
    if (!count) return ZK_OK;
    const uint32_t stride = out[0].struct_size;
    if (!abi_bytes(out, who)) return ZK_ERR_INVALID;
    for (size_t i = 0; i < count && i < (size_t)K_COUNT; ++i) {
        zk_kernel_stat* o = reinterpret_cast<zk_kernel_stat*>(reinterpret_cast<char*>(out) + i * stride);
        o->struct_size = stride;
        if (int rc = abi_put(o, src[i], who)) return rc;
    }
    return ZK_OK;
}

int zk_kernel_stats(zk_ctx* c, zk_kernel_stat* out, size_t count, int reset) {
    if (!c || (!out && count)) return fail(ZK_ERR_INVALID, "zk_kernel_stats: null argument");
    collect_kernel_stats(c);
    if (int rc = put_kernel_stats(out, count, c->kstat, "zk_kernel_stats")) return rc;
    if (reset) for (int i = 0; i < K_COUNT; ++i) c->kstat[i] = zk_kernel_stat{};
    return ZK_OK;
}

int zk_trace_fibsq(uint32_t a0, uint32_t a1, size_t count, uint32_t* out) {
    if (!out && count) return fail(ZK_ERR_INVALID, "zk_trace_fibsq: out is null");
    if (count > 0) out[0] = a0 % P;
    if (count > 1) out[1] = a1 % P;
    for (size_t i = 2; i < count; ++i)
        out[i] = add(mulmod(out[i - 2], out[i - 2]), mulmod(out[i - 1], out[i - 1]));
    return ZK_OK;
}

int zk_trace_upload(zk_ctx* c, const uint32_t* trace, size_t count) {
    if (!c || !trace) return fail(ZK_ERR_INVALID, "zk_trace_upload: null argument");
    if (count != c->n - 1) return fail(ZK_ERR_INVALID, "zk_trace_upload: expected n-1 = %zu values, got %zu", c->n - 1, count);
    for (size_t i = 0; i < count; ++i)
        if (trace[i] >= P) return fail(ZK_ERR_INVALID, "zk_trace_upload: trace[%zu] = %u is not a canonical residue", i, trace[i]);
    HIPCHK(hipSetDevice(c->device));
    HIPCHK(hipMemcpyAsync(c->d_trace, trace, count * 4, hipMemcpyHostToDevice, c->stream));
    HIPCHK(hipMemsetAsync(c->d_trace + count, 0, 4, c->stream));
    HIPCHK(hipStreamSynchronize(c->stream));
    c->first = trace[0];
    c->last = trace[count - 1];
    c->have_trace = true;
    c->have_lde = false;
    return ZK_OK;
}

int zk_lde(zk_ctx* c) {
    if (!c) return fail(ZK_ERR_INVALID, "null context");
    if (!c->have_trace) return fail(ZK_ERR_STATE, "zk_lde: no trace uploaded");
    HIPCHK(hipSetDevice(c->device));
    static const bool timing = getenv("ZK_HOST_TIMING") != nullptr;
    const double t0 = now_us();
    int rc = do_lde(c);
    if (timing) fprintf(stderr, "[zk timing] lde: enqueue of %u passes %.1f us\n", 2 * c->dom->plan.nd, now_us() - t0);
    return rc;
}

int zk_merkle_commit(zk_ctx* c, uint32_t layer, uint8_t root_out[32]) { return zk_merkle_commit_coset(c, layer, 0, root_out); }
int zk_merkle_commit_coset(zk_ctx* c, uint32_t layer, uint32_t steps, uint8_t root_out[32]) {
    if (!c || !root_out) return fail(ZK_ERR_INVALID, "zk_merkle_commit: null argument");
    if (layer > c->R + 1) return fail(ZK_ERR_INVALID, "zk_merkle_commit: layer %u out of range", layer);
    if (steps > kMaxFoldLog || (steps && layer_log(c, layer) <= steps))
        return fail(ZK_ERR_INVALID, "zk_merkle_commit_coset: need steps <= %u and at least two leaves (layer %u has 2^%u values, steps %u)", kMaxFoldLog, layer, layer_log(c, layer), steps);
    HIPCHK(hipSetDevice(c->device));
    static const bool timing = getenv("ZK_HOST_TIMING") != nullptr;
    const double t0 = now_us();
    c->skipped_trees &= ~((uint64_t)1 << layer);
    if (c->pending_top && c->pending_tree == layer) c->pending_top = false;
    int rc = settle_pending(c);
    if (rc) return rc;
    begin_proof(c);
    rc = do_merkle(c, layer, true, false, steps);
    const double t1 = now_us();
    if (!rc) rc = read_commit(c, layer, root_out);
    const double t2 = now_us();
    if (!rc && c->n_segs) { c->pending_top = true; c->pending_tree = layer; }
    if (timing)
        fprintf(stderr, "[zk timing] merkle_commit(layer %u): enqueue %.1f us, wait for the device %.1f us, host top %.1f us, scatter enqueue %.1f us\n",
                layer, t1 - t0, c->t_wait, c->t_host_hash, now_us() - t2);
    return rc;
}

int zk_compose(zk_ctx* c, const uint32_t alpha_raw[3]) {
    if (!c || !alpha_raw) return fail(ZK_ERR_INVALID, "zk_compose: null argument");
    if (!c->have_lde) return fail(ZK_ERR_STATE, "zk_compose: run zk_lde first");
    HIPCHK(hipSetDevice(c->device));
    return do_compose(c, alpha_raw);
}

int zk_fri_fold(zk_ctx* c, uint32_t round, uint32_t beta_raw) {
    if (!c) return fail(ZK_ERR_INVALID, "null context");
    if (round >= c->R) return fail(ZK_ERR_INVALID, "zk_fri_fold: round %u out of range (%u rounds)", round, c->R);
    HIPCHK(hipSetDevice(c->device));
    c->skipped_layers &= ~((uint64_t)1 << (2 + round));
    return do_fold(c, round, beta_raw);
}
int zk_fri_fold_multi(zk_ctx* c, uint32_t round, uint32_t steps, uint32_t beta_raw) {
    if (!c) return fail(ZK_ERR_INVALID, "null context");
    if (steps < 1 || steps > kMaxFoldLog) return fail(ZK_ERR_INVALID, "zk_fri_fold_multi: steps must be 1..%u (got %u)", kMaxFoldLog, steps);
    if (round >= c->R || round + steps > c->R) return fail(ZK_ERR_INVALID, "zk_fri_fold_multi: rounds %u..%u out of range (%u rounds)", round, round + steps, c->R);
    HIPCHK(hipSetDevice(c->device));
    c->skipped_layers &= ~((uint64_t)1 << (1 + round + steps));
    return dom_fold_multi(c->dom, c->d_layers + c->layer_off[1 + round], c->d_layers + c->layer_off[1 + round + steps], c->L - round, round, steps,
                          beta_raw, c->stream, prof_of(c));
}

int zk_fri_final_poly(zk_ctx* c, uint32_t layer, uint32_t bound, uint32_t* coef_out, uint32_t* high_nonzero) {
    if (!c || !coef_out || !high_nonzero) return fail(ZK_ERR_INVALID, "zk_fri_final_poly: null argument");
    if (layer < 1 || layer > c->R + 1) return fail(ZK_ERR_INVALID, "zk_fri_final_poly: layer %u out of range (FRI layers are 1..%u)", layer, c->R + 1);
    const uint32_t lg = layer_log(c, layer);
    if (lg > kFinalPolyMaxLog) return fail(ZK_ERR_INVALID, "zk_fri_final_poly: layer %u has 2^%u values, the limit is 2^%u", layer, lg, kFinalPolyMaxLog);
    if ((c->skipped_layers >> layer) & 1) return fail(ZK_ERR_STATE, "zk_fri_final_poly: layer %u was not materialised by the last proof", layer);
    HIPCHK(hipSetDevice(c->device));
    int rc = settle_pending(c);
    if (!rc) rc = final_alloc(c);
    if (!rc) rc = dom_final_poly(c->dom, c->d_layers + c->layer_off[layer], c->d_final, lg, layer - 1, bound, c->stream, prof_of(c));
    if (rc) return rc;
    HIPCHK(hipMemcpyAsync(high_nonzero, c->d_final, 4, hipMemcpyDeviceToHost, c->stream));
    HIPCHK(hipMemcpyAsync(coef_out, c->d_final + 1, ((size_t)4) << lg, hipMemcpyDeviceToHost, c->stream));
    HIPCHK(hipStreamSynchronize(c->stream));
    return ZK_OK;
}

int zk_layer_read(zk_ctx* c, uint32_t layer, size_t offset, size_t count, uint32_t* out) {
    if (!c || (!out && count)) return fail(ZK_ERR_INVALID, "zk_layer_read: null argument");
    if (layer > c->R + 1 || offset + count > layer_size(c, layer)) return fail(ZK_ERR_INVALID, "zk_layer_read: out of range");
    if ((c->skipped_layers >> layer) & 1) return fail(ZK_ERR_STATE, "zk_layer_read: layer %u was not materialised by the last proof (fold_log %u, fri_stop %u)", layer, c->fmt.fold, c->fmt.stop);
    HIPCHK(hipSetDevice(c->device));
    if (int prc = settle_pending(c)) return prc;
    HIPCHK(hipMemcpyAsync(out, c->d_layers + c->layer_off[layer] + offset, count * 4, hipMemcpyDeviceToHost, c->stream));
    HIPCHK(hipStreamSynchronize(c->stream));
    return ZK_OK;
}

int zk_layer_write(zk_ctx* c, uint32_t layer, size_t offset, size_t count, const uint32_t* in) {
    if (!c || (!in && count)) return fail(ZK_ERR_INVALID, "zk_layer_write: null argument");
    if (layer > c->R + 1 || offset + count > layer_size(c, layer)) return fail(ZK_ERR_INVALID, "zk_layer_write: out of range");
    for (size_t i = 0; i < count; ++i)
        if (in[i] >= P) return fail(ZK_ERR_INVALID, "zk_layer_write: value %zu is not a canonical residue", i);
    HIPCHK(hipSetDevice(c->device));
    HIPCHK(hipMemcpyAsync(c->d_layers + c->layer_off[layer] + offset, in, count * 4, hipMemcpyHostToDevice, c->stream));
    HIPCHK(hipStreamSynchronize(c->stream));
    if (layer == 0) c->have_lde = true;
    c->skipped_layers &= ~((uint64_t)1 << layer);
    return ZK_OK;
}

int zk_merkle_node(zk_ctx* c, uint32_t tree, size_t index, uint8_t out[32]) {
    if (!c || !out) return fail(ZK_ERR_INVALID, "zk_merkle_node: null argument");
    if (tree > c->R + 1 || index >= 2 * tree_leaves(c, tree) - 1) return fail(ZK_ERR_INVALID, "zk_merkle_node: out of range");
    if ((c->skipped_trees >> tree) & 1) return fail(ZK_ERR_STATE, "zk_merkle_node: tree %u was not built by the last proof (fold_log %u, fri_stop %u)", tree, c->fmt.fold, c->fmt.stop);
    if (index + 1 < ((size_t)1 << c->tree_cap[tree])) return fail(ZK_ERR_STATE, "zk_merkle_node: node %zu of tree %u lies above its Merkle cap (depth %u): the last proof did not build it", index, tree, c->tree_cap[tree]);
    HIPCHK(hipSetDevice(c->device));
    if (int prc = settle_pending(c)) return prc;
    HIPCHK(hipMemcpyAsync(c->h_small, c->d_trees + c->tree_off[tree] + index * 8, 32, hipMemcpyDeviceToHost, c->stream));
    HIPCHK(hipStreamSynchronize(c->stream));
    digest_words_to_bytes(c->h_small, out);
    return ZK_OK;
}

int zk_merkle_nodes(zk_ctx* c, uint32_t tree, size_t first, size_t count, uint8_t* out) {
    if (!c || (!out && count)) return fail(ZK_ERR_INVALID, "zk_merkle_nodes: null argument");
    if (tree > c->R + 1 || first > 2 * tree_leaves(c, tree) - 1 || count > 2 * tree_leaves(c, tree) - 1 - first)
        return fail(ZK_ERR_INVALID, "zk_merkle_nodes: out of range");
    if ((c->skipped_trees >> tree) & 1) return fail(ZK_ERR_STATE, "zk_merkle_nodes: tree %u was not built by the last proof (fold_log %u, fri_stop %u)", tree, c->fmt.fold, c->fmt.stop);
    if (count && first + 1 < ((size_t)1 << c->tree_cap[tree])) return fail(ZK_ERR_STATE, "zk_merkle_nodes: node %zu of tree %u lies above its Merkle cap (depth %u): the last proof did not build it", first, tree, c->tree_cap[tree]);
    HIPCHK(hipSetDevice(c->device));
    if (int prc = settle_pending(c)) return prc;
    return merkle_nodes_to_host(c->device, c->stream, c->d_trees + c->tree_off[tree], first, count, out);
}

int zk_merkle_path(zk_ctx* c, uint32_t tree, size_t leaf, uint8_t* out, size_t* path_len) {
    if (!c || !out) return fail(ZK_ERR_INVALID, "zk_merkle_path: null argument");
    if (tree > c->R + 1 || leaf >= tree_leaves(c, tree)) return fail(ZK_ERR_INVALID, "zk_merkle_path: out of range");
    if ((c->skipped_trees >> tree) & 1) return fail(ZK_ERR_STATE, "zk_merkle_path: tree %u was not built by the last proof (fold_log %u, fri_stop %u)", tree, c->fmt.fold, c->fmt.stop);
    if (c->tree_cap[tree]) return fail(ZK_ERR_STATE, "zk_merkle_path: tree %u was built down to its Merkle cap only (depth %u): a whole path does not exist", tree, c->tree_cap[tree]);
    HIPCHK(hipSetDevice(c->device));
    if (int prc = settle_pending(c)) return prc;
    std::vector<size_t> nodes;
    path_nodes(tree_leaves(c, tree), leaf, nodes);
    for (size_t i = 0; i < nodes.size(); ++i) c->h_gather_off[i] = (uint64_t)c->tree_off[tree] + (uint64_t)nodes[i] * 8;
    HIPCHK(hipMemcpyAsync(c->d_gather_off, c->h_gather_off, nodes.size() * 8, hipMemcpyHostToDevice, c->stream));
    HIPCHK(launch_gather(c->d_trees, c->d_gather_off, (uint32_t)nodes.size(), 8, c->d_gather_out, c->stream));
    HIPCHK(hipMemcpyAsync(c->h_gather_out, c->d_gather_out, nodes.size() * 32, hipMemcpyDeviceToHost, c->stream));
    HIPCHK(hipStreamSynchronize(c->stream));
    for (size_t i = 0; i < nodes.size(); ++i) digest_words_to_bytes(c->h_gather_out + 8 * i, out + 32 * i);
    if (path_len) *path_len = nodes.size();
    return ZK_OK;
}

int zk_prove_resident(zk_ctx* c, uint8_t* proof_out, size_t cap, size_t* proof_len, uint8_t state_out[32]) {
    if (!c || !proof_out || !state_out) return fail(ZK_ERR_INVALID, "zk_prove_resident: null argument");
    HIPCHK(hipSetDevice(c->device));
    Channel ch;
    int rc = prove_resident(c, ch);
    if (rc) return rc;
    const std::vector<uint8_t>& proof = ch.data;
    if (proof_len) *proof_len = proof.size();
    if (proof.size() > cap) return fail(ZK_ERR_BUFFER, "zk_prove: proof needs %zu bytes, buffer has %zu", proof.size(), cap);
    memcpy(proof_out, proof.data(), proof.size());
    memcpy(state_out, ch.state, 32);
    return ZK_OK;
}

int zk_prove_channel(zk_ctx* c, zk_channel* chan) {
    if (!c || !chan) return fail(ZK_ERR_INVALID, "zk_prove_channel: null argument");
    if (c->tail) return fail(ZK_ERR_STATE, "zk_prove_channel: FRI-tail context");
    HIPCHK(hipSetDevice(c->device));
    return prove_resident(c, chan->ch);
}

int zk_prove(zk_ctx* c, const uint32_t* trace, size_t count, uint8_t* proof_out, size_t cap, size_t* proof_len,
             uint8_t state_out[32]) {
    int rc = zk_trace_upload(c, trace, count);
    if (rc) return rc;
    return zk_prove_resident(c, proof_out, cap, proof_len, state_out);
}

int zk_prove_many(zk_ctx* const* ctxs, size_t count, uint8_t* proofs_out, size_t stride, size_t* lens_out, uint8_t* states_out) {
    if (!ctxs || !proofs_out || !lens_out || !states_out || count == 0 || count > 16)
        return fail(ZK_ERR_INVALID, "zk_prove_many: need 1..16 contexts and non-null outputs");
    for (size_t i = 0; i < count; ++i) {
        if (!ctxs[i]) return fail(ZK_ERR_INVALID, "zk_prove_many: context %zu is null", i);
        for (size_t j = 0; j < i; ++j)
            if (ctxs[j] == ctxs[i]) return fail(ZK_ERR_INVALID, "zk_prove_many: context %zu appears twice", i);
    }
    std::vector<int> rcs(count, ZK_OK);
    std::vector<std::string> errs(count);
    auto one = [&](size_t i) {
        rcs[i] = zk_prove_resident(ctxs[i], proofs_out + i * stride, stride, &lens_out[i], states_out + 32 * i);
        if (rcs[i]) errs[i] = last_error();
    };
    std::vector<std::thread> th;
    for (size_t i = 1; i < count; ++i) th.emplace_back(one, i);
    one(0);
    for (auto& t : th) t.join();
    for (size_t i = 0; i < count; ++i)
        if (rcs[i]) return fail(rcs[i], "zk_prove_many: context %zu: %s", i, errs[i].c_str());
    return ZK_OK;
}

int zk_last_transcript(const zk_ctx* c, zk_transcript_info* out) {
    if (!c || !out) return fail(ZK_ERR_INVALID, "zk_last_transcript: null argument");
    return abi_put(out, c->info, "zk_last_transcript");
}

static int verify_entry(const char* who, const uint8_t* proof, size_t len, const uint8_t* state, const ProofFormat& fmt, const uint32_t* public_last,
                        int hash_kind, int32_t* check_out, const char* replay_note, const char* reject_note) {
    if (hash_kind != ZK_HASH_SHA256 && hash_kind != ZK_HASH_FIELD && hash_kind != ZK_HASH_BLAKE2S) return fail(ZK_ERR_INVALID, "%s: unknown hash %d", who, hash_kind);
    if (fmt.fold < 1 || fmt.fold > kMaxFoldLog) return fail(ZK_ERR_INVALID, "%s: need 1 <= fold_log <= %u (got %u)", who, kMaxFoldLog, fmt.fold);
    if (fmt.cap > kMaxCapLog) return fail(ZK_ERR_INVALID, "%s: need cap_log <= %u (got %u)", who, kMaxCapLog, fmt.cap);
    int rc = state ? verify_transcript(proof, len, state, fmt) : 0;
    const bool in_replay = rc != 0;
    if (!rc) rc = verify_proof(proof, len, fmt, public_last, hash_kind);
    if (check_out) *check_out = rc;
    if (!rc) return ZK_OK;
    if (in_replay && replay_note) return fail(ZK_ERR_VERIFY, "transcript replay failed at check %d%s", rc, replay_note);
    return fail(ZK_ERR_VERIFY, "proof rejected at check %d%s", rc, reject_note);
}
static const char kProofRs[] = " (proof.rs:15-149)";

int zk_verify_ex(const uint8_t* proof, size_t len, uint32_t log_n, uint32_t log_b, uint32_t public_last, int hash_kind) {
    if (!proof) return fail(ZK_ERR_INVALID, "zk_verify: null proof");
    return verify_entry("zk_verify", proof, len, nullptr, ProofFormat{.log_n = log_n, .log_b = log_b}, &public_last, hash_kind, nullptr, nullptr, kProofRs);
}
int zk_verify(const uint8_t* proof, size_t len, uint32_t log_n, uint32_t log_b, uint32_t public_last) {
    return zk_verify_ex(proof, len, log_n, log_b, public_last, ZK_HASH_SHA256);
}
int zk_verify_queries(const uint8_t* proof, size_t len, const uint8_t* state, uint32_t log_n, uint32_t log_b, uint32_t public_last,
                      int hash_kind, uint32_t n_queries) {
    if (!proof) return fail(ZK_ERR_INVALID, "zk_verify_queries: null proof");
    return verify_entry("zk_verify_queries", proof, len, state, ProofFormat{.log_n = log_n, .log_b = log_b, .q = n_queries}, &public_last, hash_kind, nullptr, "", kProofRs);
}
int zk_verify_strict(const uint8_t* proof, size_t len, const uint8_t state[32], uint32_t log_n, uint32_t log_b, uint32_t public_last) {
    if (!proof || !state) return fail(ZK_ERR_INVALID, "zk_verify_strict: null argument");
    return verify_entry("zk_verify", proof, len, state, ProofFormat{.log_n = log_n, .log_b = log_b}, &public_last, ZK_HASH_SHA256, nullptr,
                        " (challenge not derived from the transcript, or final state mismatch)", kProofRs);
}
int zk_verify_grind(const uint8_t* proof, size_t len, const uint8_t* state, uint32_t log_n, uint32_t log_b, uint32_t public_last,
                    int hash_kind, uint32_t n_queries, uint32_t grind_bits, int32_t* check_out) {
    if (!proof || !check_out) return fail(ZK_ERR_INVALID, "zk_verify_check: null argument");
    return verify_entry("zk_verify_check", proof, len, state, ProofFormat{.log_n = log_n, .log_b = log_b, .q = n_queries, .grind = grind_bits}, &public_last, hash_kind,
                        check_out, nullptr, "");
}
int zk_verify_check(const uint8_t* proof, size_t len, const uint8_t* state, uint32_t log_n, uint32_t log_b, uint32_t public_last,
                    int hash_kind, uint32_t n_queries, int32_t* check_out) {
    if (hash_kind == ZK_HASH_BLAKE2S) return fail(ZK_ERR_INVALID, "zk_verify_check: BLAKE2s (hash 2) proofs are verified by zk_verify_stop");
    return zk_verify_grind(proof, len, state, log_n, log_b, public_last, hash_kind, n_queries, 0, check_out);
}
int zk_verify_fold(const uint8_t* proof, size_t len, const uint8_t* state, uint32_t log_n, uint32_t log_b, uint32_t public_last,
                   int hash_kind, uint32_t n_queries, uint32_t grind_bits, uint32_t fold_log, int32_t* check_out) {
    if (!proof || !check_out) return fail(ZK_ERR_INVALID, "zk_verify_fold: null argument");
    if (hash_kind == ZK_HASH_BLAKE2S) return fail(ZK_ERR_INVALID, "zk_verify_fold: BLAKE2s (hash 2) proofs are verified by zk_verify_stop");
    return verify_entry("zk_verify_fold", proof, len, state, ProofFormat{.log_n = log_n, .log_b = log_b, .q = n_queries, .grind = grind_bits, .fold = fold_log},
                        &public_last, hash_kind, check_out, nullptr, "");
}
int zk_verify_coset(const uint8_t* proof, size_t len, const uint8_t* state, uint32_t log_n, uint32_t log_b, uint32_t public_last,
                    int hash_kind, uint32_t n_queries, uint32_t grind_bits, uint32_t fold_log, int32_t* check_out) {
    if (!proof || !check_out) return fail(ZK_ERR_INVALID, "zk_verify_coset: null argument");
    return verify_entry("zk_verify_coset", proof, len, state,
                        ProofFormat{.log_n = log_n, .log_b = log_b, .q = n_queries, .grind = grind_bits, .fold = fold_log, .coset = true}, &public_last, hash_kind,
                        check_out, nullptr, "");
}
int zk_verify_stop(const uint8_t* proof, size_t len, const uint8_t* state, uint32_t log_n, uint32_t log_b, uint32_t public_last,
                   int hash_kind, uint32_t n_queries, uint32_t grind_bits, uint32_t fold_log, int coset_leaves, uint32_t stop_log, int32_t* check_out) {
    if (!proof || !check_out) return fail(ZK_ERR_INVALID, "zk_verify_stop: null argument");
    return verify_entry("zk_verify_stop", proof, len, state,
                        ProofFormat{.log_n = log_n, .log_b = log_b, .q = n_queries, .grind = grind_bits, .fold = fold_log, .coset = coset_leaves != 0, .stop = stop_log},
                        &public_last, hash_kind, check_out, nullptr, "");
}
int zk_verify_cap(const uint8_t* proof, size_t len, const uint8_t* state, uint32_t log_n, uint32_t log_b, uint32_t public_last,
                  int hash_kind, uint32_t n_queries, uint32_t grind_bits, uint32_t fold_log, int coset_leaves, uint32_t stop_log, uint32_t cap_log,
                  int32_t* check_out) {
    if (!proof || !check_out) return fail(ZK_ERR_INVALID, "zk_verify_cap: null argument");
    return verify_entry("zk_verify_cap", proof, len, state,
                        ProofFormat{.log_n = log_n, .log_b = log_b, .q = n_queries, .grind = grind_bits, .fold = fold_log, .coset = coset_leaves != 0, .stop = stop_log,
                                    .cap = cap_log},
                        &public_last, hash_kind, check_out, nullptr, "");
}
int zk_verify_shared(const uint8_t* proof, size_t len, const uint8_t* state, uint32_t log_n, uint32_t log_b, const uint32_t* public_last,
                     uint32_t log_batch, int hash_kind, uint32_t n_queries, uint32_t grind_bits, uint32_t fold_log, int coset_leaves, uint32_t stop_log,
                     uint32_t cap_log, int32_t* check_out) {
    if (!proof || !check_out || !public_last) return fail(ZK_ERR_INVALID, "zk_verify_shared: null argument");
    if (log_batch < 1 || log_batch > kMaxSharedLog) {
        *check_out = -1;
        return fail(ZK_ERR_INVALID, "zk_verify_shared: need 1 <= log_batch <= %u (got %u)", kMaxSharedLog, log_batch);
    }
    return verify_entry("zk_verify_shared", proof, len, state,
                        ProofFormat{.log_n = log_n, .log_b = log_b, .q = n_queries, .grind = grind_bits, .fold = fold_log, .coset = coset_leaves != 0, .stop = stop_log,
                                    .cap = cap_log, .lb = log_batch},
                        public_last, hash_kind, check_out, nullptr, "");
}
int zk_verify_shared_rows(const uint8_t* proof, size_t len, const uint8_t* state, uint32_t log_n, uint32_t log_b, const uint32_t* public_last,
                          uint32_t log_batch, int hash_kind, uint32_t n_queries, uint32_t grind_bits, uint32_t fold_log, int coset_leaves, uint32_t stop_log,
                          uint32_t cap_log, int row_leaves, int32_t* check_out) {
    if (!row_leaves)
        return zk_verify_shared(proof, len, state, log_n, log_b, public_last, log_batch, hash_kind, n_queries, grind_bits, fold_log, coset_leaves, stop_log, cap_log,
                                check_out);
    if (!proof || !check_out || !public_last) return fail(ZK_ERR_INVALID, "zk_verify_shared_rows: null argument");
    if (log_batch < 1 || log_batch > kMaxSharedLog) {
        *check_out = -1;
        return fail(ZK_ERR_INVALID, "zk_verify_shared_rows: row leaves need 1 <= log_batch <= %u (got %u)", kMaxSharedLog, log_batch);
    }
    if (hash_kind == ZK_HASH_BLAKE2S) {
        *check_out = -1;
        return fail(ZK_ERR_INVALID, "zk_verify_shared_rows: no BLAKE2s (hash 2) row leaves: no prover makes such a proof");
    }
    return verify_entry("zk_verify_shared_rows", proof, len, state,
                        ProofFormat{.log_n = log_n, .log_b = log_b, .q = n_queries, .grind = grind_bits, .fold = fold_log, .coset = coset_leaves != 0, .stop = stop_log,
                                    .cap = cap_log, .lb = log_batch, .rows = true},
                        public_last, hash_kind, check_out, nullptr, "");
}

size_t zk_proof_size(size_t data_len) { return 48 + data_len; }
size_t zk_proof_data_len_fold(uint32_t log_n, uint32_t log_b, uint32_t n_queries, uint32_t grind_bits, uint32_t fold_log) {
    if (fold_log < 1 || fold_log > kMaxFoldLog) return 0;
    return ProofFormat{.log_n = log_n, .log_b = log_b, .q = n_queries, .grind = grind_bits, .fold = fold_log}.data_len();
}
size_t zk_proof_data_len_coset(uint32_t log_n, uint32_t log_b, uint32_t n_queries, uint32_t grind_bits, uint32_t fold_log) {
    if (fold_log < 1 || fold_log > kMaxFoldLog) return 0;
    return ProofFormat{.log_n = log_n, .log_b = log_b, .q = n_queries, .grind = grind_bits, .fold = fold_log, .coset = true}.data_len();
}
size_t zk_proof_data_len_stop(uint32_t log_n, uint32_t log_b, uint32_t n_queries, uint32_t grind_bits, uint32_t fold_log, int coset_leaves, uint32_t stop_log) {
    if (fold_log < 1 || fold_log > kMaxFoldLog || !stop_ok(log_n, log_b, stop_log)) return 0;
    return ProofFormat{.log_n = log_n, .log_b = log_b, .q = n_queries, .grind = grind_bits, .fold = fold_log, .coset = coset_leaves != 0, .stop = stop_log}.data_len();
}
size_t zk_proof_data_len_cap(uint32_t log_n, uint32_t log_b, uint32_t n_queries, uint32_t grind_bits, uint32_t fold_log, int coset_leaves, uint32_t stop_log,
                             uint32_t cap_log) {
    if (fold_log < 1 || fold_log > kMaxFoldLog || !stop_ok(log_n, log_b, stop_log) || cap_log > kMaxCapLog) return 0;
    return ProofFormat{.log_n = log_n, .log_b = log_b, .q = n_queries, .grind = grind_bits, .fold = fold_log, .coset = coset_leaves != 0, .stop = stop_log, .cap = cap_log}
        .data_len();
}
size_t zk_proof_data_len_shared(uint32_t log_n, uint32_t log_b, uint32_t n_queries, uint32_t grind_bits, uint32_t fold_log, int coset_leaves, uint32_t stop_log,
                                uint32_t cap_log, uint32_t log_batch) {
    if (fold_log < 1 || fold_log > kMaxFoldLog || !stop_ok(log_n, log_b, stop_log) || cap_log > kMaxCapLog || log_batch > kMaxSharedLog) return 0;
    return ProofFormat{.log_n = log_n, .log_b = log_b, .q = n_queries, .grind = grind_bits, .fold = fold_log, .coset = coset_leaves != 0, .stop = stop_log, .cap = cap_log,
                       .lb = log_batch}
        .data_len();
}
size_t zk_proof_data_len_shared_rows(uint32_t log_n, uint32_t log_b, uint32_t n_queries, uint32_t grind_bits, uint32_t fold_log, int coset_leaves, uint32_t stop_log,
                                     uint32_t cap_log, uint32_t log_batch, int row_leaves) {
    if (fold_log < 1 || fold_log > kMaxFoldLog || !stop_ok(log_n, log_b, stop_log) || cap_log > kMaxCapLog || log_batch > kMaxSharedLog) return 0;
    if (row_leaves && log_batch < 1) return 0;
    return ProofFormat{.log_n = log_n, .log_b = log_b, .q = n_queries, .grind = grind_bits, .fold = fold_log, .coset = coset_leaves != 0, .stop = stop_log, .cap = cap_log,
                       .lb = log_batch, .rows = row_leaves != 0}
        .data_len();
}
size_t zk_proof_data_len_grind(uint32_t log_n, uint32_t log_b, uint32_t n_queries, uint32_t grind_bits) {
    return zk_proof_data_len_fold(log_n, log_b, n_queries, grind_bits, 1);
}
size_t zk_proof_data_len_queries(uint32_t log_n, uint32_t log_b, uint32_t n_queries) { return zk_proof_data_len_fold(log_n, log_b, n_queries, 0, 1); }
size_t zk_proof_data_len(uint32_t log_n, uint32_t log_b) { return zk_proof_data_len_fold(log_n, log_b, 1, 0, 1); }

int zk_compute_root_from_path_ex(uint32_t element, size_t index, const uint8_t* path, size_t path_len, uint8_t out[32], int hash_kind) {
    if ((!path && path_len) || !out || path_len > 62 || hash_kind < ZK_HASH_SHA256 || hash_kind > ZK_HASH_BLAKE2S)
        return fail(ZK_ERR_INVALID, "zk_compute_root_from_path: bad argument");
    compute_root_from_path(element, index, path, path_len, out, hash_kind);
    return ZK_OK;
}
int zk_compute_root_from_coset(const uint32_t* values, uint32_t s, size_t leaf, const uint8_t* path, size_t path_len, uint8_t out[32], int hash_kind) {
    if (!values || (!path && path_len) || !out || path_len > 62 || hash_kind < ZK_HASH_SHA256 || hash_kind > ZK_HASH_BLAKE2S || (s != 1 && s != 2 && s != 4 && s != 8))
        return fail(ZK_ERR_INVALID, "zk_compute_root_from_coset: bad argument");
    compute_root_from_coset(values, s, leaf, path, path_len, out, hash_kind);
    return ZK_OK;
}
int zk_compute_root_from_path(uint32_t element, size_t index, const uint8_t* path, size_t path_len, uint8_t out[32]) {
    return zk_compute_root_from_path_ex(element, index, path, path_len, out, ZK_HASH_SHA256);
}


int zk_tail_create(int device, uint32_t log_n_tail, uint32_t log_b, uint32_t shift, zk_ctx** out) {
    if (!out) return fail(ZK_ERR_INVALID, "zk_tail_create: out is null");
    *out = nullptr;
    if (log_n_tail < 1 || log_b < 1 || log_b > 5 || log_n_tail + log_b > 30)
        return fail(ZK_ERR_INVALID, "zk_tail_create: bad sizes (%u, %u)", log_n_tail, log_b);
    return ctx_make(device, log_n_tail, log_b, shift, true, out);
}

int zk_tail_run(zk_ctx* c, const uint32_t* d_layer0, void* src_stream, zk_channel* chan, int hash_kind,
                uint32_t* betas_out, uint8_t* roots_out, uint32_t* free_term_out) {
    if (hash_kind == ZK_HASH_BLAKE2S) return fail(ZK_ERR_INVALID, "zk_tail_run: %s", kNoBlake2s);
    if (!c || !c->tail || !d_layer0 || !chan || !betas_out || !roots_out || !free_term_out)
        return fail(ZK_ERR_INVALID, "zk_tail_run: bad argument");
    if (hash_kind != ZK_HASH_SHA256 && hash_kind != ZK_HASH_FIELD) return fail(ZK_ERR_INVALID, "zk_tail_run: unknown hash %d", hash_kind);
    HIPCHK(hipSetDevice(c->device));
    c->hash = hash_kind;
    HIPCHK(hipStreamSynchronize((hipStream_t)src_stream));
    HIPCHK(hipMemcpyAsync(c->d_layers + c->layer_off[1], d_layer0, c->N * 4, hipMemcpyDeviceToDevice, c->stream));
    Channel& ch = chan->ch;
    uint8_t root[32];
    int rc;
    begin_proof(c);
    if ((rc = do_merkle(c, 1, true))) return rc;
    if ((rc = read_commit(c, 1, root))) return rc;
    ch.commit_hash(root);
    memcpy(roots_out, root, 32);
    for (uint32_t r = 0; r < c->R; ++r) {
        uint32_t beta = betas_out[r] = ch.get_u32();
        if ((rc = fri_round_commit(c, r, beta, root))) return rc;
        ch.commit_hash(root);
        memcpy(roots_out + 32 * (r + 1), root, 32);
    }
    if ((rc = last_layer_value(c, free_term_out))) return rc;
    return flush_host_parts(c);
}

int zk_tail_open(zk_ctx* c, size_t x, uint32_t* vals_out, uint8_t* paths_out) {
    if (!c || !c->tail || !vals_out || !paths_out) return fail(ZK_ERR_INVALID, "zk_tail_open: bad argument");
    int rc = tail_open_begin(c, x);
    return rc ? rc : tail_open_end(c, vals_out, paths_out);
}
int zk_channel_new(zk_channel** out) {
    if (!out) return fail(ZK_ERR_INVALID, "null argument");
    *out = new (std::nothrow) zk_channel();
    return *out ? ZK_OK : fail(ZK_ERR_NOMEM, "out of host memory");
}
int zk_channel_free(zk_channel* ch) { delete ch; return ZK_OK; }
int zk_channel_import(zk_channel* ch, const uint8_t state[32], const uint8_t* data, size_t n) {
    if (!ch || !state || (!data && n)) return fail(ZK_ERR_INVALID, "null argument");
    memcpy(ch->ch.state, state, 32);
    ch->ch.data.assign(data, data + n);
    return ZK_OK;
}
int zk_channel_commit(zk_channel* ch, const uint8_t* bytes, size_t n) {
    if (!ch || (!bytes && n)) return fail(ZK_ERR_INVALID, "null argument");
    ch->ch.commit_bytes(bytes, n);
    return ZK_OK;
}
int zk_channel_get_u32(zk_channel* ch, uint32_t* out) {
    if (!ch || !out) return fail(ZK_ERR_INVALID, "null argument");
    *out = ch->ch.get_u32();
    return ZK_OK;
}
int zk_channel_state(const zk_channel* ch, uint8_t out[32]) {
    if (!ch || !out) return fail(ZK_ERR_INVALID, "null argument");
    memcpy(out, ch->ch.state, 32);
    return ZK_OK;
}
size_t zk_channel_data_len(const zk_channel* ch) { return ch ? ch->ch.data.size() : 0; }
int zk_channel_data(const zk_channel* ch, uint8_t* out, size_t cap) {
    if (!ch || !out) return fail(ZK_ERR_INVALID, "null argument");
    if (ch->ch.data.size() > cap) return fail(ZK_ERR_BUFFER, "buffer too small");
    memcpy(out, ch->ch.data.data(), ch->ch.data.size());
    return ZK_OK;
}

static Profiler g_dev_prof;
static zk_kernel_stat g_dev_kstat[K_COUNT] = {};
static Profiler* dev_prof() { return g_dev_prof.mask ? &g_dev_prof : nullptr; }

int zk_dev_set_profiling(uint32_t class_mask) {
    g_dev_prof.mask = class_mask & ((1u << K_COUNT) - 1u);
    return ZK_OK;
}
int zk_dev_kernel_stats(zk_kernel_stat* out, size_t count, int reset) {
    if (!out && count) return fail(ZK_ERR_INVALID, "zk_dev_kernel_stats: null argument");
    for (auto& r : g_dev_prof.recs) {
        float ms = 0;
        (void)hipEventSynchronize(r.b);
        (void)hipEventElapsedTime(&ms, r.a, r.b);
        g_dev_kstat[r.cls].launches += 1; g_dev_kstat[r.cls].ms += ms; g_dev_kstat[r.cls].bytes += r.bytes; g_dev_kstat[r.cls].ops += r.ops;
        g_dev_prof.pool.push_back(r.a); g_dev_prof.pool.push_back(r.b);
    }
    g_dev_prof.recs.clear();
    if (int rc = put_kernel_stats(out, count, g_dev_kstat, "zk_dev_kernel_stats")) return rc;
    if (reset) for (int i = 0; i < K_COUNT; ++i) g_dev_kstat[i] = zk_kernel_stat{};
    return ZK_OK;
}

int zk_dom_create(int device, uint32_t log_n, uint32_t log_b, uint32_t shift, int fold_only, zk_dom** out) {
    if (!out) return fail(ZK_ERR_INVALID, "zk_dom_create: out is null");
    return dom_make(device, log_n, log_b, shift, fold_only != 0, nullptr, out);
}
int zk_dom_destroy(zk_dom* d) {
    if (d) { (void)hipSetDevice(d->device); dom_free(d); }
    return ZK_OK;
}
int zk_dev_lde(const zk_dom* d, const uint32_t* d_trace, uint32_t* d_coef, uint32_t* d_out, void* stream) {
    if (!d || !d_trace || !d_coef || !d_out) return fail(ZK_ERR_INVALID, "zk_dev_lde: null argument");
    if (!d->d_inv_xm1) return fail(ZK_ERR_STATE, "zk_dev_lde: fold-only domain");
    HIPCHK(hipSetDevice(d->device));
    return dom_lde(d, d_trace, d_coef, d_out, (hipStream_t)stream, dev_prof());
}
int zk_dev_compose(const zk_dom* d, const uint32_t* d_f, uint32_t* d_cp, uint32_t first, uint32_t last,
                   const uint32_t alpha_raw[3], void* stream) {
    if (!d || !d_f || !d_cp || !alpha_raw) return fail(ZK_ERR_INVALID, "zk_dev_compose: null argument");
    if (!d->d_inv_xm1) return fail(ZK_ERR_STATE, "zk_dev_compose: fold-only domain");
    HIPCHK(hipSetDevice(d->device));
    return dom_compose(d, d_f, d_cp, first, last, alpha_raw, (hipStream_t)stream, dev_prof());
}
int zk_dev_fri_fold(const zk_dom* d, const uint32_t* d_in, uint32_t* d_out, uint32_t log_m, uint32_t round,
                    uint32_t beta_raw, void* stream) {
    if (!d || !d_in || !d_out) return fail(ZK_ERR_INVALID, "zk_dev_fri_fold: null argument");
    HIPCHK(hipSetDevice(d->device));
    return dom_fold(d, d_in, d_out, log_m, round, beta_raw, (hipStream_t)stream, dev_prof());
}
int zk_dev_fri_fold_multi(const zk_dom* d, const uint32_t* d_in, uint32_t* d_out, uint32_t log_m, uint32_t round, uint32_t steps,
                          uint32_t beta_raw, void* stream) {
    if (!d || !d_in || !d_out) return fail(ZK_ERR_INVALID, "zk_dev_fri_fold_multi: null argument");
    if (steps < 1 || steps > kMaxFoldLog) return fail(ZK_ERR_INVALID, "zk_dev_fri_fold_multi: steps must be 1..%u (got %u)", kMaxFoldLog, steps);
    if (round + steps > d->log_n || log_m + round != d->L)
        return fail(ZK_ERR_INVALID, "zk_dev_fri_fold_multi: layer 2^%u, rounds %u..%u do not fit a domain of %u rounds", log_m, round, round + steps, d->log_n);
    HIPCHK(hipSetDevice(d->device));
    return dom_fold_multi(d, d_in, d_out, log_m, round, steps, beta_raw, (hipStream_t)stream, dev_prof());
}
int zk_dev_fri_fold_multi_batch(const zk_dom* d, const uint32_t* d_in, uint32_t* d_out, uint32_t log_m, uint32_t round, uint32_t steps,
                                const uint32_t* d_beta_raw, uint32_t* d_work, uint32_t batch, void* stream) {
    if (!d || !d_in || !d_out || !d_beta_raw || !d_work) return fail(ZK_ERR_INVALID, "zk_dev_fri_fold_multi_batch: null argument");
    if (steps < 1 || steps > kMaxFoldLog) return fail(ZK_ERR_INVALID, "zk_dev_fri_fold_multi_batch: steps must be 1..%u (got %u)", kMaxFoldLog, steps);
    if (round + steps > d->log_n || log_m + round != d->L)
        return fail(ZK_ERR_INVALID, "zk_dev_fri_fold_multi_batch: layer 2^%u, rounds %u..%u do not fit a domain of %u rounds", log_m, round, round + steps, d->log_n);
    if (batch < 1 || ((uint64_t)batch << log_m) > ((uint64_t)1 << 32))
        return fail(ZK_ERR_INVALID, "zk_dev_fri_fold_multi_batch: need batch >= 1 and batch * 2^log_m <= 2^32 (got %u, log_m %u)", batch, log_m);
    HIPCHK(hipSetDevice(d->device));
    return dom_fold_multi_batch(d, d_in, d_out, log_m, round, steps, d_beta_raw, 1, d_work, batch, (hipStream_t)stream, dev_prof());
}
int zk_dev_trace_fibsq_batch(const uint32_t* d_a0, const uint32_t* d_a1, uint32_t batch, uint32_t count, uint32_t* d_out, void* stream) {
    if ((batch && (!d_a0 || !d_a1 || !d_out))) return fail(ZK_ERR_INVALID, "zk_dev_trace_fibsq_batch: null argument");
    HIPCHK(launch_trace_fibsq_batch(d_a0, d_a1, batch, count, d_out, (hipStream_t)stream));
    return ZK_OK;
}
int zk_trace_fibsq_batch_host(int device, const uint32_t* a0, const uint32_t* a1, uint32_t batch, uint32_t count, uint32_t* out) {
    if (batch && (!a0 || !a1 || !out)) return fail(ZK_ERR_INVALID, "zk_trace_fibsq_batch_host: null argument");
    if (!batch || !count) return ZK_OK;
    HIPCHK(hipSetDevice(device));
    uint32_t *d0 = nullptr, *d1 = nullptr, *dout = nullptr;
    HIPCHK(hipMalloc(&d0, batch * 4)); HIPCHK(hipMalloc(&d1, batch * 4));
    hipError_t e = hipMalloc(&dout, (size_t)batch * count * 4);
    int rc = ZK_OK;
    if (e != hipSuccess) rc = fail(ZK_ERR_NOMEM, "hipMalloc failed");
    if (!rc && (hipMemcpy(d0, a0, batch * 4, hipMemcpyHostToDevice) != hipSuccess || hipMemcpy(d1, a1, batch * 4, hipMemcpyHostToDevice) != hipSuccess)) rc = fail(ZK_ERR_HIP, "H2D failed");
    if (!rc && launch_trace_fibsq_batch(d0, d1, batch, count, dout, nullptr) != hipSuccess) rc = fail(ZK_ERR_HIP, "launch failed");
    if (!rc && hipMemcpy(out, dout, (size_t)batch * count * 4, hipMemcpyDeviceToHost) != hipSuccess) rc = fail(ZK_ERR_HIP, "D2H failed");
    (void)hipFree(d0); (void)hipFree(d1); if (dout) (void)hipFree(dout);
    return rc;
}
int zk_dev_interleave(const uint32_t* d_in, uint32_t* d_out, uint32_t log_parts, uint32_t log_cnt, void* stream) {
    if (!d_in || !d_out || log_parts + log_cnt > 31) return fail(ZK_ERR_INVALID, "zk_dev_interleave: bad argument");
    HIPCHK(launch_interleave(d_in, d_out, log_parts, log_cnt, (hipStream_t)stream));
    return ZK_OK;
}
int zk_dev_gather(const uint32_t* d_src, const uint64_t* d_offsets, uint32_t count, uint32_t words, uint32_t* d_out, void* stream) {
    if (!d_src || (!d_offsets && count) || (!d_out && count)) return fail(ZK_ERR_INVALID, "zk_dev_gather: null argument");
    HIPCHK(launch_gather(d_src, d_offsets, count, words, d_out, (hipStream_t)stream, dev_prof()));
    return ZK_OK;
}

int zk_dev_merkle_build_ex(const uint32_t* d_vals, uint32_t log_m, uint32_t* d_nodes, void* stream, int hash_kind) {
    if (!d_vals || !d_nodes || log_m > 30 || hash_kind < ZK_HASH_SHA256 || hash_kind > ZK_HASH_BLAKE2S) return fail(ZK_ERR_INVALID, "zk_dev_merkle_build: bad argument");
    HIPCHK(launch_merkle_build(d_vals, log_m, d_nodes, (hipStream_t)stream, dev_prof(), MailArgs{}, hash_kind));
    return ZK_OK;
}
int zk_dev_merkle_build_rows(const uint32_t* d_vals, uint32_t log_len, uint32_t log_batch, uint32_t* d_nodes, void* stream, int hash_kind) {
    if (!d_vals || !d_nodes || log_batch < 1 || log_batch > kMaxSharedLog || log_len < 1 || log_len + log_batch > 30)
        return fail(ZK_ERR_INVALID, "zk_dev_merkle_build_rows: need 1 <= log_batch <= %u, 1 <= log_len and log_len + log_batch <= 30", kMaxSharedLog);
    if (hash_kind != ZK_HASH_SHA256 && hash_kind != ZK_HASH_FIELD) return fail(ZK_ERR_INVALID, "zk_dev_merkle_build_rows: row leaves take hash 0 or 1 (got %d)", hash_kind);
    HIPCHK(launch_merkle_build_rows(d_vals, log_len, log_batch, d_nodes, (hipStream_t)stream, dev_prof(), MailArgs{}, hash_kind));
    return ZK_OK;
}
int zk_row_leaf_hash(const uint32_t* values, uint32_t m, int hash_kind, uint8_t out[32]) {
    if (!values || !out || m < 1 || m > (1u << kMaxSharedLog) || (m & (m - 1))) return fail(ZK_ERR_INVALID, "zk_row_leaf_hash: need a power of two 1 <= m <= %u values", 1u << kMaxSharedLog);
    if (hash_kind != ZK_HASH_SHA256 && hash_kind != ZK_HASH_FIELD) return fail(ZK_ERR_INVALID, "zk_row_leaf_hash: row leaves take hash 0 or 1 (got %d)", hash_kind);
    host_coset_leaf_hash(values, m, out, hash_kind);
    return ZK_OK;
}
int zk_dev_merkle_build_interleaved(const uint32_t* d_recv, uint32_t log_parts, uint32_t log_cnt, uint32_t* d_nodes, void* stream, int hash_kind) {
    if (hash_kind == ZK_HASH_BLAKE2S) return fail(ZK_ERR_INVALID, "zk_dev_merkle_build_interleaved: %s", kNoBlake2s);
    if (!d_recv || !d_nodes || log_parts + log_cnt > 30 || (hash_kind != 0 && hash_kind != 1))
        return fail(ZK_ERR_INVALID, "zk_dev_merkle_build_interleaved: bad argument");
    HIPCHK(launch_merkle_build_interleaved(d_recv, log_parts, log_cnt, d_nodes, (hipStream_t)stream, dev_prof(), hash_kind));
    return ZK_OK;
}
struct zk_committer {
    int device = 0;
    uint32_t* h_mail = nullptr;
    uint32_t* d_mail = nullptr;
    uint32_t* d_counter = nullptr;
    bool counters_dirty = false;
    uint32_t* h_stage = nullptr;
    uint32_t* d_stage = nullptr;
    uint32_t seq = 0, top = 0;
    static constexpr uint32_t kSlots = 40;
    static constexpr size_t kSlotWords = (size_t)16 << kHostTopSingle;
    bool lazy = false;
    uint32_t* base = nullptr;
    uint32_t n_pending = 0;
    double pending_words = 0;
    hipEvent_t stage_free = nullptr;
    bool stage_busy = false;
    int (*poll)(void*) = nullptr;
    void* poll_user = nullptr;
    double timeout_s = 30.0;
};
extern "C++" {
namespace zk { namespace impl {
void committer_set_poll(zk_committer* k, int (*poll)(void*), void* user, double timeout_s) {
    if (k) { k->poll = poll; k->poll_user = user; if (timeout_s > 0) k->timeout_s = timeout_s; }
}
} }
}
int zk_committer_destroy(zk_committer* k) {
    if (!k) return ZK_OK;
    (void)hipSetDevice(k->device);
    (void)hipDeviceSynchronize();
    if (k->stage_free) (void)hipEventDestroy(k->stage_free);
    if (k->h_mail) (void)hipHostFree(k->h_mail);
    if (k->h_stage) (void)hipHostFree(k->h_stage);
    if (k->d_counter) (void)hipFree(k->d_counter);
    delete k;
    return ZK_OK;
}
int zk_committer_create(int device, zk_committer** out) {
    if (!out) return fail(ZK_ERR_INVALID, "zk_committer_create: out is null");
    *out = nullptr;
    HIPCHK(hipSetDevice(device));
    zk_committer* k = new (std::nothrow) zk_committer();
    if (!k) return fail(ZK_ERR_NOMEM, "out of host memory");
    k->device = device;
    static_assert(zk_committer::kSlots * zk_committer::kSlotWords >= ((size_t)16 << kMaxHostLog), "staging: one eager commit fits");
    static_assert(zk_committer::kSlotWords >= 8 * ((size_t)2 << kHostTopSingle) - 8, "staging: a lazy commit's nodes AND posted digests fit its own slot");
    const size_t stage_bytes = zk_committer::kSlots * zk_committer::kSlotWords * 4 + zk_committer::kSlots * sizeof(ScatterSeg);
    hipError_t e = hipHostMalloc((void**)&k->h_mail, kMailValsOff * 4, hipHostMallocMapped | hipHostMallocCoherent);
    if (e == hipSuccess) e = hipHostGetDevicePointer((void**)&k->d_mail, k->h_mail, 0);
    if (e == hipSuccess) e = hipHostMalloc((void**)&k->h_stage, stage_bytes, hipHostMallocMapped | hipHostMallocCoherent);
    if (e == hipSuccess) e = hipHostGetDevicePointer((void**)&k->d_stage, k->h_stage, 0);
    if (e == hipSuccess) e = hipMalloc((void**)&k->d_counter, 64);
    if (e == hipSuccess) e = hipMemset(k->d_counter, 0, 64);
    if (e == hipSuccess) e = hipEventCreateWithFlags(&k->stage_free, hipEventDisableTiming);
    if (e != hipSuccess) { zk_committer_destroy(k); return fail(ZK_ERR_HIP, "zk_committer_create: %s", hipGetErrorString(e)); }
    memset(k->h_mail, 0, kMailValsOff * 4);
    k->top = host_sha_available() ? 8 : 0;
    *out = k;
    return ZK_OK;
}
int zk_committer_set_top(zk_committer* k, uint32_t top_log) {
    if (!k) return fail(ZK_ERR_INVALID, "null committer");
    if (top_log > kHostTopSingle) return fail(ZK_ERR_INVALID, "zk_committer_set_top: need top_log <= %u (one thread reduces the top)", kHostTopSingle);
    k->top = top_log;
    return ZK_OK;
}
static uint32_t* committer_counter(zk_committer* k, hipStream_t s) {
    if (k->counters_dirty) { (void)hipMemsetAsync(k->d_counter, 0, 64, s); k->counters_dirty = false; }
    return k->d_counter;
}
static ScatterSeg* committer_segs(zk_committer* k, bool device) {
    return reinterpret_cast<ScatterSeg*>((device ? k->d_stage : k->h_stage) + zk_committer::kSlots * zk_committer::kSlotWords);
}
static int committer_flush_impl(zk_committer* k, hipStream_t s) {
    if (!k->n_pending) return ZK_OK;
    HIPCHK(launch_scatter(k->d_stage, committer_segs(k, true), k->n_pending, k->pending_words, k->base, nullptr, s, dev_prof()));
    HIPCHK(hipEventRecord(k->stage_free, s));
    k->stage_busy = true;
    k->n_pending = 0;
    k->pending_words = 0;
    return ZK_OK;
}
static int committer_collect(zk_committer* k, const MailArgs& m, uint32_t* d_nodes, hipStream_t s, uint8_t root_out[32]) {
    int rc = wait_flag(k->h_mail, m.seq, s, k->poll, k->poll_user, k->timeout_s);
    if (rc) { k->counters_dirty = true; return rc; }
    if (!m.top) { digest_words_to_bytes(k->h_mail + kMailDigests, root_out); return ZK_OK; }
    const size_t cnt = (size_t)1 << m.top;
    const bool lazy = k->lazy && k->base && d_nodes >= k->base;
    if (lazy && k->n_pending == zk_committer::kSlots)
        if ((rc = committer_flush_impl(k, s))) return rc;
    if (k->stage_busy && (!lazy || k->n_pending == 0)) {
        HIPCHK(hipEventSynchronize(k->stage_free));
        k->stage_busy = false;
    }
    const uint32_t slot = lazy ? k->n_pending : 0u;
    uint32_t* nodes = k->h_stage + (size_t)slot * zk_committer::kSlotWords;
    memcpy(nodes + 8 * (cnt - 1), k->h_mail + kMailDigests, cnt * 32);
    host_sha_reduce(nodes, m.top);
    digest_words_to_bytes(nodes, root_out);
    ScatterSeg* seg = committer_segs(k, false) + slot;
    *seg = ScatterSeg{(uint64_t)slot * zk_committer::kSlotWords, lazy ? (uint64_t)(d_nodes - k->base) : 0u, (uint32_t)((cnt - 1) * 8), 0};
    if (lazy) {
        k->n_pending += 1;
        k->pending_words += (double)seg->words;
        return ZK_OK;
    }
    HIPCHK(launch_scatter(k->d_stage, committer_segs(k, true), 1, (double)seg->words, d_nodes, nullptr, s, dev_prof()));
    HIPCHK(hipEventRecord(k->stage_free, s));
    k->stage_busy = true;
    return ZK_OK;
}
extern "C++" {
namespace zk { namespace impl {
void committer_set_lazy(zk_committer* k, uint32_t* trees_base) {
    if (k) { k->lazy = trees_base != nullptr; k->base = trees_base; }
}
int committer_flush(zk_committer* k, hipStream_t s) {
    if (!k) return ZK_OK;
    HIPCHK(hipSetDevice(k->device));
    return committer_flush_impl(k, s);
}
void committer_drop_pending(zk_committer* k) {
    if (k) { k->n_pending = 0; k->pending_words = 0; }
}
} }
}

int zk_dev_merkle_commit(zk_committer* k, const uint32_t* d_src, uint32_t log_parts, uint32_t log_cnt, uint32_t* d_nodes, void* stream,
                         int hash_kind, uint8_t root_out[32]) {
    if (hash_kind == ZK_HASH_BLAKE2S) return fail(ZK_ERR_INVALID, "zk_dev_merkle_commit: %s", kNoBlake2s);
    if (!k || !d_src || !d_nodes || !root_out || log_parts + log_cnt > 30 || (hash_kind != 0 && hash_kind != 1))
        return fail(ZK_ERR_INVALID, "zk_dev_merkle_commit: bad argument");
    HIPCHK(hipSetDevice(k->device));
    const uint32_t log_m = log_parts + log_cnt;
    hipStream_t s = (hipStream_t)stream;
    MailArgs m;
    m.mailbox = k->d_mail;
    m.seq = ++k->seq;
    m.counter = committer_counter(k, s);
    m.top = (hash_kind == 0 && k->top && log_m > k->top) ? k->top : 0;
    if (log_parts) HIPCHK(launch_merkle_build_interleaved(d_src, log_parts, log_cnt, d_nodes, s, dev_prof(), hash_kind, m));
    else HIPCHK(launch_merkle_build(d_src, log_m, d_nodes, s, dev_prof(), m, hash_kind));
    return committer_collect(k, m, d_nodes, s, root_out);
}

extern "C++" {
namespace zk {
namespace impl {
int dev_compose_block_commit(zk_committer* k, const zk_dom* glob, ComposeBlockArgs geom, uint32_t first, uint32_t last, const uint32_t alpha_raw[3],
                             uint32_t* d_nodes, hipStream_t s, int hash_kind, uint8_t root_out[32], int (*enqueued)(void*), void* user) {
    if (hash_kind == ZK_HASH_BLAKE2S) return fail(ZK_ERR_INVALID, "dev_compose_block_commit: %s", kNoBlake2s);
    if (!k || !glob || !geom.a.f || !geom.a.inv_xm1 || !geom.halo || !d_nodes || !root_out || (hash_kind != 0 && hash_kind != 1) ||
        geom.log_m > 30 || geom.lg + geom.log_cnt > geom.log_m)
        return fail(ZK_ERR_INVALID, "dev_compose_block_commit: bad argument");
    if (((size_t)1 << geom.log_m) < 2 * glob->B || geom.halo_stride < (2 * glob->B) >> geom.lg)
        return fail(ZK_ERR_INVALID, "dev_compose_block_commit: a block of 2^%u leaves is shorter than the 2B = %zu taps", geom.log_m, 2 * glob->B);
    HIPCHK(hipSetDevice(k->device));
    const uint32_t* f = geom.a.f;
    const uint32_t* inv = geom.a.inv_xm1;
    int rc = compose_args(glob, f, nullptr, first, last, alpha_raw, geom.a);
    if (rc) return rc;
    geom.a.inv_xm1 = inv;
    MailArgs m;
    m.mailbox = k->d_mail;
    m.seq = ++k->seq;
    m.counter = committer_counter(k, s);
    m.top = (hash_kind == 0 && k->top && geom.log_m > k->top) ? k->top : 0;
    HIPCHK(launch_compose_block_merkle(geom, d_nodes, s, dev_prof(), m, hash_kind));
    if (enqueued)
        if ((rc = enqueued(user))) return rc;
    return committer_collect(k, m, d_nodes, s, root_out);
}
}
}
}

int zk_dev_merkle_commit_finish(zk_committer* k, uint32_t* d_nodes, uint32_t log_m, uint32_t log_chunks, void* stream, int hash_kind,
                                uint8_t root_out[32]) {
    if (hash_kind == ZK_HASH_BLAKE2S) return fail(ZK_ERR_INVALID, "zk_dev_merkle_commit_finish: %s", kNoBlake2s);
    if (!k || !d_nodes || !root_out || log_m > 30 || log_chunks > 10 || log_chunks > log_m || (hash_kind != 0 && hash_kind != 1))
        return fail(ZK_ERR_INVALID, "zk_dev_merkle_commit_finish: bad argument");
    HIPCHK(hipSetDevice(k->device));
    hipStream_t s = (hipStream_t)stream;
    MailArgs m;
    m.mailbox = k->d_mail;
    m.seq = ++k->seq;
    m.counter = committer_counter(k, s);
    m.top = (hash_kind == 0 && k->top && merkle_finish_start_depth(log_m, log_chunks) > k->top) ? k->top : 0;
    HIPCHK(launch_merkle_finish(d_nodes, log_m, log_chunks, s, dev_prof(), hash_kind, m));
    return committer_collect(k, m, d_nodes, s, root_out);
}

int zk_dev_merkle_build_chunk(const uint32_t* d_recv, uint32_t log_parts, uint32_t log_cnt, uint32_t* d_nodes, uint32_t log_m,
                              uint32_t chunk, void* stream, int hash_kind) {
    if (hash_kind == ZK_HASH_BLAKE2S) return fail(ZK_ERR_INVALID, "zk_dev_merkle_build_chunk: %s", kNoBlake2s);
    if (!d_recv || !d_nodes || log_m > 30 || log_parts + log_cnt > log_m || (hash_kind != 0 && hash_kind != 1) ||
        chunk >= (1u << (log_m - log_parts - log_cnt)))
        return fail(ZK_ERR_INVALID, "zk_dev_merkle_build_chunk: bad argument");
    HIPCHK(launch_merkle_build_chunk(d_recv, log_parts, log_cnt, d_nodes, log_m, chunk, (hipStream_t)stream, dev_prof(), hash_kind));
    return ZK_OK;
}
int zk_dev_merkle_finish(uint32_t* d_nodes, uint32_t log_m, uint32_t log_chunks, void* stream, int hash_kind) {
    if (hash_kind == ZK_HASH_BLAKE2S) return fail(ZK_ERR_INVALID, "zk_dev_merkle_finish: %s", kNoBlake2s);
    if (!d_nodes || log_m > 30 || log_chunks > 10 || log_chunks > log_m || (hash_kind != 0 && hash_kind != 1))
        return fail(ZK_ERR_INVALID, "zk_dev_merkle_finish: bad argument");
    HIPCHK(launch_merkle_finish(d_nodes, log_m, log_chunks, (hipStream_t)stream, dev_prof(), hash_kind));
    return ZK_OK;
}
int zk_dev_set_merkle_latency_log(uint32_t log_nodes) {
    if (!set_merkle_latency_log(log_nodes)) return fail(ZK_ERR_INVALID, "zk_dev_set_merkle_latency_log: need 12 <= log_nodes <= 24 (0 = default)");
    return ZK_OK;
}
int zk_dev_merkle_build(const uint32_t* d_vals, uint32_t log_m, uint32_t* d_nodes, void* stream) {
    return zk_dev_merkle_build_ex(d_vals, log_m, d_nodes, stream, ZK_HASH_SHA256);
}

int zk_dev_merkle_node(const uint32_t* d_nodes, size_t index, uint8_t out[32], void* stream) {
    if (!d_nodes || !out) return fail(ZK_ERR_INVALID, "zk_dev_merkle_node: null argument");
    uint32_t w[8];
    HIPCHK(hipMemcpyAsync(w, d_nodes + index * 8, 32, hipMemcpyDeviceToHost, (hipStream_t)stream));
    HIPCHK(hipStreamSynchronize((hipStream_t)stream));
    digest_words_to_bytes(w, out);
    return ZK_OK;
}

int zk_merkle_build_host(int device, const uint32_t* vals, size_t m, uint8_t* nodes_out) {
    return zk_merkle_build_host_ex(device, vals, m, nodes_out, ZK_HASH_SHA256);
}

int zk_merkle_build_host_ex(int device, const uint32_t* vals, size_t m, uint8_t* nodes_out, int hash_kind) {
    if (!vals || !nodes_out) return fail(ZK_ERR_INVALID, "zk_merkle_build_host: null argument");
    if (hash_kind < ZK_HASH_SHA256 || hash_kind > ZK_HASH_BLAKE2S) return fail(ZK_ERR_INVALID, "zk_merkle_build_host: unknown hash %d", hash_kind);
    if (m == 0 || (m & (m - 1)) || m > ((size_t)1 << 30))
        return fail(ZK_ERR_INVALID, "zk_merkle_build_host: size %zu is not a power of two (merkle.rs:18)", m);
    uint32_t log_m = 0;
    while (((size_t)1 << log_m) < m) ++log_m;
    HIPCHK(hipSetDevice(device));
    uint32_t *d_vals = nullptr, *d_nodes = nullptr;
    size_t words = (2 * m - 1) * 8;
    HIPCHK(hipMalloc(&d_vals, m * 4));
    hipError_t e = hipMalloc(&d_nodes, words * 4);
    if (e != hipSuccess) { (void)hipFree(d_vals); return fail(ZK_ERR_NOMEM, "hipMalloc failed"); }
    int rc = ZK_OK;
    std::vector<uint32_t> host(words);
    do {
        if (hipMemcpy(d_vals, vals, m * 4, hipMemcpyHostToDevice) != hipSuccess) { rc = fail(ZK_ERR_HIP, "H2D failed"); break; }
        if (launch_merkle_build(d_vals, log_m, d_nodes, nullptr, nullptr, MailArgs{}, hash_kind) != hipSuccess) { rc = fail(ZK_ERR_HIP, "merkle launch failed"); break; }
        if (hipMemcpy(host.data(), d_nodes, words * 4, hipMemcpyDeviceToHost) != hipSuccess) { rc = fail(ZK_ERR_HIP, "D2H failed: %s", hipGetErrorString(hipGetLastError())); break; }
    } while (0);
    (void)hipFree(d_vals); (void)hipFree(d_nodes);
    if (rc) return rc;
    for (size_t i = 0; i < 2 * m - 1; ++i) digest_words_to_bytes(host.data() + 8 * i, nodes_out + 32 * i);
    return ZK_OK;
}

int zk_probe_hash_chain(int device, int hash_kind, uint32_t waves_per_simd, uint32_t hashes, uint32_t launches, zk_chain_probe* out) {
    if (!out || hash_kind < ZK_HASH_SHA256 || hash_kind > ZK_HASH_BLAKE2S || waves_per_simd < 1 || waves_per_simd > 8 || !hashes || !launches)
        return fail(ZK_ERR_INVALID, "zk_probe_hash_chain: bad argument");
    if (!abi_bytes(out, "zk_probe_hash_chain")) return ZK_ERR_INVALID;
    zk_chain_probe* const user_out = out;
    zk_chain_probe res{};
    out = &res;
    HIPCHK(hipSetDevice(device));
    hipDeviceProp_t prop;
    HIPCHK(hipGetDeviceProperties(&prop, device));
    const uint32_t cus = (uint32_t)prop.multiProcessorCount, blocks = cus * waves_per_simd;
    uint32_t* d_out = nullptr;
    unsigned long long* d_rec = nullptr;
    HIPCHK(hipMalloc(&d_out, (size_t)blocks * 256 * 4));
    hipError_t e = hipMalloc(&d_rec, (size_t)blocks * 4 * 16);
    if (e != hipSuccess) { (void)hipFree(d_out); return fail(ZK_ERR_NOMEM, "hipMalloc failed"); }
    hipEvent_t e0 = nullptr, e1 = nullptr;
    int rc = ZK_OK;
    std::vector<unsigned long long> rec((size_t)blocks * 8);
    do {
        if (hipEventCreate(&e0) != hipSuccess || hipEventCreate(&e1) != hipSuccess) { rc = fail(ZK_ERR_HIP, "hipEventCreate failed"); break; }
        if (launch_hash_chain_probe(hash_kind, blocks, d_out, 3u, hashes, d_rec, nullptr) != hipSuccess || hipDeviceSynchronize() != hipSuccess) {
            rc = fail(ZK_ERR_HIP, "probe launch failed"); break;
        }
        (void)hipEventRecord(e0, nullptr);
        for (uint32_t r = 0; r < launches; ++r) (void)launch_hash_chain_probe(hash_kind, blocks, d_out, 12345u + r, hashes, d_rec, nullptr);
        (void)hipEventRecord(e1, nullptr);
        if (hipEventSynchronize(e1) != hipSuccess) { rc = fail(ZK_ERR_HIP, "probe failed: %s", hipGetErrorString(hipGetLastError())); break; }
        float ms = 0;
        (void)hipEventElapsedTime(&ms, e0, e1);
        if (hipMemcpy(rec.data(), d_rec, rec.size() * 8, hipMemcpyDeviceToHost) != hipSuccess) { rc = fail(ZK_ERR_HIP, "D2H failed"); break; }
        std::vector<double> ghz;
        for (size_t i = 0; i + 1 < rec.size(); i += 2)
            if (rec[i + 1]) ghz.push_back((double)rec[i] / (double)rec[i + 1] * 0.1);
        std::sort(ghz.begin(), ghz.end());
        out->ms = ms;
        out->ns_per_hash_per_simd = (double)ms * 1e6 / ((double)launches * waves_per_simd * hashes);
        out->clock_ghz = ghz.empty() ? 0.0 : ghz[ghz.size() / 2];
        out->waves_per_simd = waves_per_simd; out->launches = launches; out->hashes = hashes; out->cus = cus;
    } while (0);
    if (e0) (void)hipEventDestroy(e0);
    if (e1) (void)hipEventDestroy(e1);
    (void)hipFree(d_out); (void)hipFree(d_rec);
    return rc ? rc : abi_put(user_out, res, "zk_probe_hash_chain");
}

int zk_probe_fieldhash_forms(int device, uint32_t count, uint32_t seed, uint32_t* mismatches, uint32_t* first_bad) {
    if (!mismatches || count == 0 || count > (1u << 26)) return fail(ZK_ERR_INVALID, "zk_probe_fieldhash_forms: bad argument");
    HIPCHK(hipSetDevice(device));
    uint32_t* d_res = nullptr;
    HIPCHK(hipMalloc(&d_res, 8));
    const uint32_t init[2] = {0u, 0xFFFFFFFFu};
    int rc = ZK_OK;
    uint32_t res[2] = {0, 0};
    if (hipMemcpy(d_res, init, 8, hipMemcpyHostToDevice) != hipSuccess || launch_fieldhash_forms((count + 255) / 256, seed, d_res, nullptr) != hipSuccess ||
        hipMemcpy(res, d_res, 8, hipMemcpyDeviceToHost) != hipSuccess)
        rc = fail(ZK_ERR_HIP, "zk_probe_fieldhash_forms: %s", hipGetErrorString(hipGetLastError()));
    (void)hipFree(d_res);
    if (rc) return rc;
    *mismatches = res[0];
    if (first_bad) *first_bad = res[1];
    return ZK_OK;
}

int zk_ntt_host(int device, uint32_t* data, uint32_t log_m, int inverse) {
    if (!data || log_m < 1 || log_m > 30) return fail(ZK_ERR_INVALID, "zk_ntt_host: bad argument");
    size_t m = (size_t)1 << log_m;
    for (size_t i = 0; i < m; ++i)
        if (data[i] >= P) return fail(ZK_ERR_INVALID, "zk_ntt_host: data[%zu] is not a canonical residue", i);
    HIPCHK(hipSetDevice(device));
    uint32_t root = root_of_unity(log_m);
    DevTable T;
    int rc = build_table(inverse ? invmod(root) : root, log_m, &T);
    if (rc) return rc;
    Plan pl = make_plan(log_m);
    uint32_t *d_a = nullptr, *d_b = nullptr;
    HIPCHK(hipMalloc(&d_a, m * 4));
    HIPCHK(hipMalloc(&d_b, m * 4));
    do {
        if (hipMemcpy(d_a, data, m * 4, hipMemcpyHostToDevice) != hipSuccess) { rc = fail(ZK_ERR_HIP, "H2D failed"); break; }
        uint32_t* res = d_a;
        if (inverse) {
            if ((rc = run_dif(d_a, d_a, log_m, pl, T.view(), log_m, to_mont(invmod((uint32_t)(m % P))), nullptr))) break;
            if (launch_digit_reverse(d_a, d_b, log_m, pl.nd, pl.bits, 1, nullptr) != hipSuccess) { rc = fail(ZK_ERR_HIP, "launch failed"); break; }
            res = d_b;
        } else {
            if (launch_digit_reverse(d_a, d_b, log_m, pl.nd, pl.bits, 0, nullptr) != hipSuccess) { rc = fail(ZK_ERR_HIP, "launch failed"); break; }
            if ((rc = run_dit(d_b, log_m, pl, T.view(), log_m, nullptr))) break;
            res = d_b;
        }
        if (hipMemcpy(data, res, m * 4, hipMemcpyDeviceToHost) != hipSuccess) { rc = fail(ZK_ERR_HIP, "D2H failed: %s", hipGetErrorString(hipGetLastError())); break; }
    } while (0);
    (void)hipFree(d_a); (void)hipFree(d_b);
    free_table(&T);
    return rc;
}

int zk_lde_host(int device, const uint32_t* trace, uint32_t log_n, uint32_t log_b, uint32_t* out) {
    if (!trace || !out) return fail(ZK_ERR_INVALID, "zk_lde_host: null argument");
    zk_ctx* c = nullptr;
    int rc = zk_ctx_create(device, log_n, log_b, &c);
    if (rc) return rc;
    rc = zk_trace_upload(c, trace, c->n - 1);
    if (!rc) rc = zk_lde(c);
    if (!rc) rc = zk_layer_read(c, 0, 0, c->N, out);
    zk_ctx_destroy(c);
    return rc;
}

}
```

Measured before the change: 2.920 billion.

## Keep host Merkle levels in AVX-512 registers and interleave paired SHA streams

Host Merkle reduction now keeps digests of a subtree of up to 2^10 leaves in transposed AVX-512 form across levels, using permutes instead of reloading and retransposing each level. On AMD CPUs two 16-lane SHA-256 streams are interleaved to hide instruction latency. The host-side FRI fold is vectorised with AVX-512 Montgomery arithmetic, its twiddle tables are precomputed at context creation, and the fold is fused with leaf hashing and tree building. It also drops the tail_vals vector copies in favour of pointers and adds per-turn timing instrumentation, at the cost of more code paths and register pressure.

```diff
diff --git a/zkstark_amd/csrc/host_sha.cpp b/zkstark_amd/csrc/host_sha.cpp
--- a/zkstark_amd/csrc/host_sha.cpp
+++ b/zkstark_amd/csrc/host_sha.cpp
@@ -1,6 +1,11 @@
 #include "host_sha.hpp"
 
 #include <atomic>
+
+#if defined(__HIPCC__)
+#include <hip/hip_runtime.h>
+#endif
+#include "field.hpp"
 
 #if !defined(__HIP_DEVICE_COMPILE__)
 #include <immintrin.h>
@@ -27,6 +32,8 @@
 bool g_cpu_has_sha = false, g_cpu_has_x16 = false;
 std::atomic<bool> g_have_sha{false}, g_have_x16{false};
 std::atomic<bool> g_want_x16{true};
+bool g_cpu_pair = false;
+std::atomic<bool> g_pair{false};
 
 inline uint32_t rotr(uint32_t x, int n) { return (x >> n) | (x << (32 - n)); }
 
@@ -37,6 +44,8 @@
         g_cpu_has_x16 = g_cpu_has_sha && __builtin_cpu_supports("avx512f");
         g_have_sha = g_cpu_has_sha;
         g_have_x16 = g_cpu_has_x16;
+        g_cpu_pair = g_cpu_has_x16 && __builtin_cpu_is("amd");
+        g_pair = g_cpu_pair;
         uint32_t w[64] = {0x80000000u};
         w[15] = 512u;
         for (int t = 16; t < 64; ++t) {
@@ -211,31 +220,52 @@
     }
 }
 
+#define ZK_X16_ROUND(msg, t, S)                                                                                                       \
+    do {                                                                                                                              \
+        __m512i wk;                                                                                                                   \
+        if (msg) {                                                                                                                    \
+            if ((t) >= 16) {                                                                                                          \
+                const __m512i w15 = w##S[((t) + 1) & 15], w2 = w##S[((t) + 14) & 15];                                                 \
+                const __m512i x0 = ZK_XOR3(ZK_ROR(w15, 7), ZK_ROR(w15, 18), _mm512_srli_epi32(w15, 3));                               \
+                const __m512i x1 = ZK_XOR3(ZK_ROR(w2, 17), ZK_ROR(w2, 19), _mm512_srli_epi32(w2, 10));                                \
+                w##S[(t) & 15] = _mm512_add_epi32(_mm512_add_epi32(w##S[(t) & 15], x0), _mm512_add_epi32(w##S[((t) + 9) & 15], x1));  \
+            }                                                                                                                         \
+            wk = _mm512_add_epi32(w##S[(t) & 15], _mm512_set1_epi32((int)K[t]));                                                      \
+        } else {                                                                                                                      \
+            wk = _mm512_set1_epi32((int)PADKW[t]);                                                                                    \
+        }                                                                                                                             \
+        const __m512i S1 = ZK_XOR3(ZK_ROR(e##S, 6), ZK_ROR(e##S, 11), ZK_ROR(e##S, 25));                                              \
+        const __m512i t1 = _mm512_add_epi32(_mm512_add_epi32(h##S, S1), _mm512_add_epi32(_mm512_ternarylogic_epi32(e##S, f##S, g##S, 0xCA), wk)); \
+        const __m512i S0 = ZK_XOR3(ZK_ROR(a##S, 2), ZK_ROR(a##S, 13), ZK_ROR(a##S, 22));                                              \
+        const __m512i t2 = _mm512_add_epi32(S0, _mm512_ternarylogic_epi32(a##S, b##S, c##S, 0xE8));                                   \
+        h##S = g##S; g##S = f##S; f##S = e##S; e##S = _mm512_add_epi32(d##S, t1); d##S = c##S; c##S = b##S; b##S = a##S;              \
+        a##S = _mm512_add_epi32(t1, t2);                                                                                              \
+    } while (0)
+#define ZK_X16_BEGIN(S, st) __m512i a##S = st[0], b##S = st[1], c##S = st[2], d##S = st[3], e##S = st[4], f##S = st[5], g##S = st[6], h##S = st[7]
+#define ZK_X16_END(S, st)                                                                                                             \
+    do {                                                                                                                              \
+        st[0] = _mm512_add_epi32(st[0], a##S); st[1] = _mm512_add_epi32(st[1], b##S); st[2] = _mm512_add_epi32(st[2], c##S);          \
+        st[3] = _mm512_add_epi32(st[3], d##S); st[4] = _mm512_add_epi32(st[4], e##S); st[5] = _mm512_add_epi32(st[5], f##S);          \
+        st[6] = _mm512_add_epi32(st[6], g##S); st[7] = _mm512_add_epi32(st[7], h##S);                                                 \
+    } while (0)
 template <bool MSG>
-ZK_X16_TARGET inline void rounds_x16(__m512i st[8], __m512i w[16]) {
-    __m512i a = st[0], b = st[1], c = st[2], d = st[3], e = st[4], f = st[5], g = st[6], h = st[7];
+ZK_X16_TARGET inline void rounds_x16(__m512i st[8], __m512i w0[16]) {
+    ZK_X16_BEGIN(0, st);
+#pragma GCC unroll 64
+    for (int t = 0; t < 64; ++t) ZK_X16_ROUND(MSG, t, 0);
+    ZK_X16_END(0, st);
+}
+template <bool MSG>
+ZK_X16_TARGET inline void rounds_x16x2(__m512i sa[8], __m512i w0[16], __m512i sb[8], __m512i w1[16]) {
+    ZK_X16_BEGIN(0, sa);
+    ZK_X16_BEGIN(1, sb);
 #pragma GCC unroll 64
     for (int t = 0; t < 64; ++t) {
-        __m512i wk;
-        if (MSG) {
-            if (t >= 16) {
-                const __m512i w15 = w[(t + 1) & 15], w2 = w[(t + 14) & 15];
-                const __m512i s0 = ZK_XOR3(ZK_ROR(w15, 7), ZK_ROR(w15, 18), _mm512_srli_epi32(w15, 3));
-                const __m512i s1 = ZK_XOR3(ZK_ROR(w2, 17), ZK_ROR(w2, 19), _mm512_srli_epi32(w2, 10));
-                w[t & 15] = _mm512_add_epi32(_mm512_add_epi32(w[t & 15], s0), _mm512_add_epi32(w[(t + 9) & 15], s1));
-            }
-            wk = _mm512_add_epi32(w[t & 15], _mm512_set1_epi32((int)K[t]));
-        } else {
-            wk = _mm512_set1_epi32((int)PADKW[t]);
-        }
-        const __m512i S1 = ZK_XOR3(ZK_ROR(e, 6), ZK_ROR(e, 11), ZK_ROR(e, 25));
-        const __m512i t1 = _mm512_add_epi32(_mm512_add_epi32(h, S1), _mm512_add_epi32(_mm512_ternarylogic_epi32(e, f, g, 0xCA), wk));
-        const __m512i S0 = ZK_XOR3(ZK_ROR(a, 2), ZK_ROR(a, 13), ZK_ROR(a, 22));
-        const __m512i t2 = _mm512_add_epi32(S0, _mm512_ternarylogic_epi32(a, b, c, 0xE8));
-        h = g; g = f; f = e; e = _mm512_add_epi32(d, t1); d = c; c = b; b = a; a = _mm512_add_epi32(t1, t2);
-    }
-    st[0] = _mm512_add_epi32(st[0], a); st[1] = _mm512_add_epi32(st[1], b); st[2] = _mm512_add_epi32(st[2], c); st[3] = _mm512_add_epi32(st[3], d);
-    st[4] = _mm512_add_epi32(st[4], e); st[5] = _mm512_add_epi32(st[5], f); st[6] = _mm512_add_epi32(st[6], g); st[7] = _mm512_add_epi32(st[7], h);
+        ZK_X16_ROUND(MSG, t, 0);
+        ZK_X16_ROUND(MSG, t, 1);
+    }
+    ZK_X16_END(0, sa);
+    ZK_X16_END(1, sb);
 }
 ZK_X16_TARGET inline void store_x16(const __m512i st[8], uint32_t* out) {
     __m512i r[16];
@@ -271,19 +301,152 @@
     for (; i < cnt; ++i) inner_ni(child + 16 * i, child + 16 * i + 8, out + 8 * i);
 }
 
-ZK_SHA_TARGET void reduce_ni(uint32_t* nodes, uint32_t depth) {
-    for (uint32_t d = depth; d-- > 0;) {
-        const size_t base = ((size_t)1 << d) - 1, child = ((size_t)2 << d) - 1, cnt = (size_t)1 << d;
-        inner_run(nodes + 8 * child, nodes + 8 * base, cnt);
-    }
-}
-
-ZK_SHA_TARGET void reduce_sub_ni(uint32_t* nodes, uint32_t depth, uint32_t top, size_t sub) {
+constexpr uint32_t kLaneLog = 10;
+
+ZK_X16_TARGET __attribute__((noinline)) void node_x16(__m512i w[16], __m512i st[8]) {
+    for (int i = 0; i < 8; ++i) st[i] = _mm512_set1_epi32((int)IV[i]);
+    rounds_x16<true>(st, w);
+    rounds_x16<false>(st, w);
+}
+ZK_X16_TARGET __attribute__((noinline)) void node_x16x2(__m512i wa[16], __m512i sa[8], __m512i wb[16], __m512i sb[8]) {
+    for (int i = 0; i < 8; ++i) sa[i] = sb[i] = _mm512_set1_epi32((int)IV[i]);
+    rounds_x16x2<true>(sa, wa, sb, wb);
+    rounds_x16x2<false>(sa, wa, sb, wb);
+}
+ZK_X16_TARGET __attribute__((noinline)) void leaf_rows_x16(__m512i v, __m512i st[8]) {
+    __m512i w[16];
+    w[0] = v;
+    w[1] = _mm512_set1_epi32((int)0x80000000u);
+    for (int i = 2; i < 15; ++i) w[i] = _mm512_setzero_si512();
+    w[15] = _mm512_set1_epi32(32);
+    for (int i = 0; i < 8; ++i) st[i] = _mm512_set1_epi32((int)IV[i]);
+    rounds_x16<true>(st, w);
+}
+ZK_X16_TARGET __attribute__((noinline)) void leaf_rows_x16x2(__m512i va, __m512i sa[8], __m512i vb, __m512i sb[8]) {
+    __m512i wa[16], wb[16];
+    wa[0] = va; wb[0] = vb;
+    wa[1] = wb[1] = _mm512_set1_epi32((int)0x80000000u);
+    for (int i = 2; i < 15; ++i) wa[i] = wb[i] = _mm512_setzero_si512();
+    wa[15] = wb[15] = _mm512_set1_epi32(32);
+    for (int i = 0; i < 8; ++i) sa[i] = sb[i] = _mm512_set1_epi32((int)IV[i]);
+    rounds_x16x2<true>(sa, wa, sb, wb);
+}
+template <bool HEAP>
+ZK_X16_TARGET inline void rows_x16(const uint32_t* child, const __m512i* cur, size_t b, __m512i w[16]) {
+    if (HEAP) {
+        for (int n = 0; n < 16; ++n) w[n] = _mm512_loadu_si512((const void*)(child + 256 * b + 16 * n));
+        transpose16(w);
+    } else {
+        const __m512i even = _mm512_setr_epi32(0, 2, 4, 6, 8, 10, 12, 14, 16, 18, 20, 22, 24, 26, 28, 30);
+        const __m512i odd = _mm512_setr_epi32(1, 3, 5, 7, 9, 11, 13, 15, 17, 19, 21, 23, 25, 27, 29, 31);
+        const __m512i* a = cur + 16 * b;
+        for (int t = 0; t < 8; ++t) {
+            w[t] = _mm512_permutex2var_epi32(a[t], even, a[8 + t]);
+            w[8 + t] = _mm512_permutex2var_epi32(a[t], odd, a[8 + t]);
+        }
+    }
+}
+template <bool HEAP>
+ZK_X16_TARGET void level_x16(const uint32_t* child, uint32_t* out, __m512i* cur, size_t nb) {
+    size_t b = 0;
+    if (g_pair)
+        for (; b + 2 <= nb; b += 2) {
+            __m512i wa[16], wb[16];
+            rows_x16<HEAP>(child, cur, b, wa);
+            rows_x16<HEAP>(child, cur, b + 1, wb);
+            node_x16x2(wa, cur + 8 * b, wb, cur + 8 * b + 8);
+            store_x16(cur + 8 * b, out + 128 * b);
+            store_x16(cur + 8 * b + 8, out + 128 * b + 128);
+        }
+    for (; b < nb; ++b) {
+        __m512i w[16];
+        rows_x16<HEAP>(child, cur, b, w);
+        node_x16(w, cur + 8 * b);
+        store_x16(cur + 8 * b, out + 128 * b);
+    }
+}
+
+ZK_X16_TARGET void lanes_up(uint32_t* nodes, __m512i* cur, uint32_t d, uint32_t top, size_t sub) {
+    size_t cnt = (size_t)1 << (d - top);
+    while (cnt >= 32) {
+        --d;
+        cnt >>= 1;
+        level_x16<false>(nodes + 8 * (((size_t)2 << d) - 1 + 2 * sub * cnt), nodes + 8 * (((size_t)1 << d) - 1 + sub * cnt), cur, cnt / 16);
+    }
+    while (d-- > top) {
+        cnt = (size_t)1 << (d - top);
+        inner_run(nodes + 8 * (((size_t)2 << d) - 1 + 2 * sub * cnt), nodes + 8 * (((size_t)1 << d) - 1 + sub * cnt), cnt);
+    }
+}
+ZK_X16_TARGET void reduce_sub_x16(uint32_t* nodes, uint32_t depth, uint32_t top, size_t sub) {
+    __m512i cur[8 << (kLaneLog - 5)];
+    const uint32_t d = depth - 1;
+    const size_t cnt = (size_t)1 << (d - top);
+    const uint32_t* child = nodes + 8 * (((size_t)2 << d) - 1 + 2 * sub * cnt);
+    uint32_t* out = nodes + 8 * (((size_t)1 << d) - 1 + sub * cnt);
+    level_x16<true>(child, out, cur, cnt / 16);
+    lanes_up(nodes, cur, d, top, sub);
+}
+
+void reduce_sub_ni(uint32_t* nodes, uint32_t depth, uint32_t top, size_t sub) {
+    if (g_have_x16) {
+        while (depth - top > kLaneLog) {
+            const uint32_t mid = depth - kLaneLog;
+            for (size_t s = 0; s < ((size_t)1 << (mid - top)); ++s) reduce_sub_x16(nodes, depth, mid, (sub << (mid - top)) + s);
+            depth = mid;
+        }
+        if (depth - top >= 5) { reduce_sub_x16(nodes, depth, top, sub); return; }
+    }
     for (uint32_t d = depth; d-- > top;) {
         const size_t cnt = (size_t)1 << (d - top);
         const size_t base = ((size_t)1 << d) - 1 + sub * cnt, child = ((size_t)2 << d) - 1 + 2 * sub * cnt;
         inner_run(nodes + 8 * child, nodes + 8 * base, cnt);
     }
+}
+void reduce_ni(uint32_t* nodes, uint32_t depth) { reduce_sub_ni(nodes, depth, 0, 0); }
+
+ZK_X16_TARGET inline __m512i add_x16(__m512i a, __m512i b) {
+    const __m512i p = _mm512_set1_epi32((int)P);
+    const __m512i nb = _mm512_sub_epi32(p, b), d = _mm512_sub_epi32(a, nb);
+    return _mm512_mask_add_epi32(d, _mm512_cmplt_epu32_mask(a, nb), d, p);
+}
+ZK_X16_TARGET inline __m512i sub_x16(__m512i a, __m512i b) {
+    const __m512i d = _mm512_sub_epi32(a, b);
+    return _mm512_mask_add_epi32(d, _mm512_cmplt_epu32_mask(a, b), d, _mm512_set1_epi32((int)P));
+}
+ZK_X16_TARGET inline __m512i mont_mul_x8(__m512i a, __m512i b) {
+    const __m512i p = _mm512_set1_epi64((long long)P);
+    const __m512i t = _mm512_mul_epu32(a, b);
+    const __m512i m = _mm512_add_epi64(t, _mm512_slli_epi64(t, 30));
+    const __m512i hi = _mm512_srli_epi64(t, 32), mp_hi = _mm512_srli_epi64(_mm512_mul_epu32(m, p), 32);
+    const __m512i r = _mm512_sub_epi64(hi, mp_hi);
+    return _mm512_mask_add_epi64(r, _mm512_cmplt_epu64_mask(hi, mp_hi), r, p);
+}
+ZK_X16_TARGET inline __m512i mont_mul_x16(__m512i a, __m512i b) {
+    const __m512i e = mont_mul_x8(a, b), o = mont_mul_x8(_mm512_srli_epi64(a, 32), _mm512_srli_epi64(b, 32));
+    return _mm512_mask_blend_epi32(0xAAAA, e, _mm512_slli_epi64(o, 32));
+}
+ZK_X16_TARGET void fold_tree_x16(const uint32_t* in, uint32_t log_half, const uint32_t* xinv_m, uint32_t cc_m, uint32_t inv2_m,
+                                 uint32_t* out, uint32_t* nodes) {
+    __m512i cur[8 << (kLaneLog - 4)];
+    const size_t half = (size_t)1 << log_half;
+    const __m512i cc = _mm512_set1_epi32((int)cc_m), inv2 = _mm512_set1_epi32((int)inv2_m);
+    const size_t nb = half / 16;
+    __m512i prev = _mm512_setzero_si512();
+    for (size_t b = 0; b < nb; ++b) {
+        const __m512i u = _mm512_loadu_si512((const void*)(in + 16 * b)), v = _mm512_loadu_si512((const void*)(in + half + 16 * b));
+        const __m512i x = _mm512_loadu_si512((const void*)(xinv_m + 16 * b));
+        const __m512i f = add_x16(mont_mul_x16(add_x16(u, v), inv2), mont_mul_x16(mont_mul_x16(sub_x16(u, v), x), cc));
+        _mm512_storeu_si512((void*)(out + 16 * b), f);
+        if (g_pair && nb > 1) {
+            if (b & 1) leaf_rows_x16x2(prev, cur + 8 * b - 8, f, cur + 8 * b);
+            prev = f;
+        } else {
+            leaf_rows_x16(f, cur + 8 * b);
+        }
+    }
+    for (size_t b = 0; b < nb; ++b) store_x16(cur + 8 * b, nodes + 8 * (half - 1 + 16 * b));
+    lanes_up(nodes, cur, log_half, 0, 0);
 }
 
 void compress_generic(uint32_t st[8], const uint32_t blk[16]) {
@@ -315,6 +478,9 @@
     g_want_x16 = on;
     g_have_x16 = on && g_have_sha.load(std::memory_order_relaxed) && g_cpu_has_x16;
 }
+
+bool host_sha_pairs() { return g_pair; }
+void host_sha_use_pairs(bool on) { g_pair = on && g_cpu_has_x16; }
 
 void host_sha_compress(uint32_t state[8], const uint32_t block[16]) {
     if (g_have_sha) compress_ni(state, block);
@@ -383,5 +549,23 @@
     }
 }
 
+void host_fold_table(uint32_t step, uint32_t log_half, uint32_t* xinv_m) {
+    const uint32_t step_m = to_mont(step);
+    uint32_t x = to_mont(1);
+    for (size_t i = 0; i < ((size_t)1 << log_half); ++i) { xinv_m[i] = x; x = mont_mul(x, step_m); }
+}
+
+void host_fold_tree(const uint32_t* in, uint32_t log_half, const uint32_t* xinv_m, uint32_t cc_m, uint32_t inv2_m, uint32_t* out,
+                    uint32_t* nodes) {
+    if (g_have_x16 && log_half >= 4 && log_half <= kLaneLog) { fold_tree_x16(in, log_half, xinv_m, cc_m, inv2_m, out, nodes); return; }
+    const size_t half = (size_t)1 << log_half;
+    for (size_t i = 0; i < half; ++i) {
+        const uint32_t u = in[i], v = in[i + half];
+        out[i] = add(mont_mul(add(u, v), inv2_m), mont_mul(mont_mul(sub(u, v), xinv_m[i]), cc_m));
+    }
+    host_sha_leaves(out, half, nodes + 8 * (half - 1));
+    host_sha_reduce(nodes, log_half);
+}
+
 }
 #endif
diff --git a/zkstark_amd/csrc/host_sha.hpp b/zkstark_amd/csrc/host_sha.hpp
--- a/zkstark_amd/csrc/host_sha.hpp
+++ b/zkstark_amd/csrc/host_sha.hpp
@@ -8,6 +8,8 @@
 void host_sha_use_extensions(bool on);
 bool host_sha_wide_available();
 void host_sha_use_wide(bool on);
+bool host_sha_pairs();
+void host_sha_use_pairs(bool on);
 void host_sha_compress(uint32_t state[8], const uint32_t block[16]);
 void host_sha_blocks(uint32_t state[8], const uint8_t* data, size_t blocks);
 void host_sha_leaf(uint32_t v, uint32_t out[8]);
@@ -16,5 +18,8 @@
 void host_sha_inner_run(const uint32_t* children, uint32_t* out, size_t cnt);
 void host_sha_reduce(uint32_t* nodes, uint32_t depth);
 void host_sha_reduce_sub(uint32_t* nodes, uint32_t depth, uint32_t top, size_t sub);
+void host_fold_table(uint32_t step, uint32_t log_half, uint32_t* xinv_m);
+void host_fold_tree(const uint32_t* in, uint32_t log_half, const uint32_t* xinv_m, uint32_t cc_m, uint32_t inv2_m, uint32_t* out,
+                    uint32_t* nodes);
 
 }
diff --git a/zkstark_amd/csrc/zkstark.hip b/zkstark_amd/csrc/zkstark.hip
--- a/zkstark_amd/csrc/zkstark.hip
+++ b/zkstark_amd/csrc/zkstark.hip
@@ -79,10 +79,15 @@
     ScatterSeg* d_segs = nullptr;
     uint32_t n_segs = 0;
     double seg_words = 0;
-    std::vector<uint32_t> tail_vals;
+    const uint32_t* tail_vals = nullptr;
     uint32_t tail_log = 0;
     bool tail_have = false;
+    std::vector<uint32_t> tail_xinv;
     double t_wait = 0, t_host_hash = 0, t_launch = 0;
+    bool timing = false;
+    struct Turn { double wait = 0, mail = 0, hash = 0, book = 0, chan = 0, launch = 0; } turn[40];
+    static constexpr uint32_t kTurnStart = 39;
+    uint32_t turn_of = kTurnStart;
     bool tail = false;
     uint32_t hinv_host = 0;
     ProofFormat fmt;
@@ -125,6 +130,15 @@
 
 Profiler* prof_of(zk_ctx* c) { return c->prof.mask ? &c->prof : nullptr; }
 
+inline double lap_now(const zk_ctx* c) { return c->timing ? now_us() : 0.0; }
+struct TurnClock {
+    zk_ctx* c;
+    double zk_ctx::Turn::*item;
+    double t0;
+    TurnClock(zk_ctx* ctx, double zk_ctx::Turn::*it) : c(ctx), item(it), t0(lap_now(ctx)) {}
+    ~TurnClock() { if (c->timing) c->turn[c->turn_of].*item += now_us() - t0; }
+};
+
 void collect_kernel_stats(zk_ctx* c) {
     for (auto& r : c->prof.recs) {
         float ms = 0;
@@ -141,6 +155,7 @@
 }
 
 int do_lde(zk_ctx* c) {
+    TurnClock clock{c, &zk_ctx::Turn::launch};
     int rc = dom_lde(c->dom, c->d_trace, c->d_coef, c->d_layers + c->layer_off[0], c->stream, prof_of(c));
     if (!rc) c->have_lde = true;
     return rc;
@@ -186,12 +201,14 @@
 }
 
 int do_merkle(zk_ctx* c, uint32_t layer, bool host = false, bool feed_tail = true, uint32_t steps = 0) {
+    TurnClock clock{c, &zk_ctx::Turn::launch};
     HIPCHK(launch_merkle_build_coset(c->d_layers + c->layer_off[layer], layer_log(c, layer), steps, c->d_trees + c->tree_off[layer], c->stream,
                                      prof_of(c), mail_of(c, layer, host, feed_tail, steps), c->hash));
     return ZK_OK;
 }
 
 int do_compose_commit(zk_ctx* c, const uint32_t alpha_raw[3]) {
+    TurnClock clock{c, &zk_ctx::Turn::launch};
     ComposeArgs a;
     int rc = compose_args(c->dom, c->d_layers + c->layer_off[0], c->d_layers + c->layer_off[1], c->first, c->last, alpha_raw, a);
     if (rc) return rc;
@@ -199,6 +216,7 @@
     return ZK_OK;
 }
 int do_fold_commit(zk_ctx* c, uint32_t round, uint32_t beta_raw) {
+    TurnClock clock{c, &zk_ctx::Turn::launch};
     FoldArgs a;
     int rc = fold_args(c->dom, c->d_layers + c->layer_off[1 + round], c->d_layers + c->layer_off[2 + round], c->L - round, round, beta_raw, a);
     if (rc) return rc;
@@ -234,14 +252,23 @@
     return ZK_OK;
 }
 
+void book_turn(zk_ctx* c, uint32_t tree, double ta, double t0, double tb, double t1) {
+    c->turn_of = tree;
+    if (!c->timing) return;
+    zk_ctx::Turn& t = c->turn[tree];
+    t.wait += t0 - ta; t.mail += tb - t0; t.hash += t1 - tb; t.book += now_us() - t1;
+}
+
 int read_commit_cap(zk_ctx* c, uint32_t tree, uint32_t H, uint32_t ce, uint8_t root[32]) {
     const size_t cnt = (size_t)1 << H, first = ((size_t)1 << ce) - 1, ncap = (size_t)1 << ce;
     uint32_t* nodes = stage_alloc(c, (2 * cnt - 1) * 8);
     if (!nodes) return fail(ZK_ERR_STATE, "host staging buffer exhausted");
+    const double ta = lap_now(c);
     int rc = wait_mail(c, c->tree_seq[tree]);
     if (rc) return rc;
     double t0 = now_us();
     memcpy(nodes + 8 * (cnt - 1), c->h_mailbox + kMailDigests, cnt * 32);
+    const double tb = lap_now(c);
     if (H > ce) {
         if (c->pool) c->pool->run(ncap, 1, [&](size_t sub) { host_sha_reduce_sub(nodes, H, ce, sub); });
         else for (size_t sub = 0; sub < ncap; ++sub) host_sha_reduce_sub(nodes, H, ce, sub);
@@ -250,13 +277,14 @@
     cd.resize(32 * ncap);
     for (size_t i = 0; i < ncap; ++i) digest_words_to_bytes(nodes + 8 * (first + i), cd.data() + 32 * i);
     memset(root, 0, 32);
-    c->t_host_hash += now_us() - t0;
-    if (c->tail_have && c->tail_log == layer_log(c, tree) && tree >= 1) {
-        c->tail_vals.assign(c->h_mailbox + kMailValsOff, c->h_mailbox + kMailValsOff + ((size_t)1 << c->tail_log));
-    }
+    const double t1 = now_us();
+    c->t_host_hash += t1 - t0;
+    if (c->tail_have && c->tail_log == layer_log(c, tree) && tree >= 1) c->tail_vals = c->h_mailbox + kMailValsOff;
     c->host_nodes[tree] = nodes;
     c->host_node_cnt[tree] = 2 * cnt - 1;
-    return H > ce ? stage_seg(c, nodes + 8 * first, c->tree_off[tree] + 8 * first, (cnt - 1 - first) * 8, 0) : (int)ZK_OK;
+    rc = H > ce ? stage_seg(c, nodes + 8 * first, c->tree_off[tree] + 8 * first, (cnt - 1 - first) * 8, 0) : (int)ZK_OK;
+    book_turn(c, tree, ta, t0, tb, t1);
+    return rc;
 }
 
 int read_commit(zk_ctx* c, uint32_t tree, uint8_t root[32]) {
@@ -266,10 +294,12 @@
     const size_t cnt = (size_t)1 << H;
     uint32_t* nodes = stage_alloc(c, (2 * cnt - 1) * 8);
     if (!nodes) return fail(ZK_ERR_STATE, "host staging buffer exhausted");
+    const double ta = lap_now(c);
     int rc = wait_mail(c, c->tree_seq[tree]);
     if (rc) return rc;
     double t0 = now_us();
     memcpy(nodes + 8 * (cnt - 1), c->h_mailbox + kMailDigests, cnt * 32);
+    const double tb = lap_now(c);
     const uint32_t sub_log = host_sub_log();
     if (H > sub_log && c->pool) {
         const uint32_t top = H - sub_log;
@@ -279,13 +309,14 @@
         host_sha_reduce(nodes, H);
     }
     digest_words_to_bytes(nodes, root);
-    c->t_host_hash += now_us() - t0;
-    if (c->tail_have && c->tail_log == layer_log(c, tree) && tree >= 1) {
-        c->tail_vals.assign(c->h_mailbox + kMailValsOff, c->h_mailbox + kMailValsOff + ((size_t)1 << c->tail_log));
-    }
+    const double t1 = now_us();
+    c->t_host_hash += t1 - t0;
+    if (c->tail_have && c->tail_log == layer_log(c, tree) && tree >= 1) c->tail_vals = c->h_mailbox + kMailValsOff;
     c->host_nodes[tree] = nodes;
     c->host_node_cnt[tree] = 2 * cnt - 1;
-    return stage_seg(c, nodes, c->tree_off[tree], (cnt - 1) * 8, 0);
+    rc = stage_seg(c, nodes, c->tree_off[tree], (cnt - 1) * 8, 0);
+    book_turn(c, tree, ta, t0, tb, t1);
+    return rc;
 }
 
 int host_fold_commit(zk_ctx* c, uint32_t round, uint32_t beta_raw, uint8_t root[32]) {
@@ -297,20 +328,13 @@
     if (!vals || !nodes) return fail(ZK_ERR_STATE, "host staging buffer exhausted");
     const zk_dom* d = c->dom;
     const uint32_t cc_m = to_mont(mulmod(beta_raw % P, d->fold_k[round]));
-    const uint32_t step_m = to_mont(powmod(c->hinv_host, (uint64_t)1 << round));
-    const uint32_t* in = c->tail_vals.data();
-    uint32_t xinv_m = to_mont(1);
-    for (size_t i = 0; i < half; ++i) {
-        uint32_t u = in[i], v = in[i + half];
-        vals[i] = add(mont_mul(add(u, v), d->inv2_mont), mont_mul(mont_mul(sub(u, v), xinv_m), cc_m));
-        xinv_m = mont_mul(xinv_m, step_m);
-    }
-    host_sha_leaves(vals, half, nodes + 8 * (half - 1));
-    host_sha_reduce(nodes, log_out);
+    host_fold_tree(c->tail_vals, log_out, c->tail_xinv.data() + (half - 1), cc_m, d->inv2_mont, vals, nodes);
     digest_words_to_bytes(nodes, root);
-    c->tail_vals.assign(vals, vals + half);
+    c->tail_vals = vals;
     c->tail_log = log_out;
-    c->t_host_hash += now_us() - t_begin;
+    const double t_end = now_us();
+    c->t_host_hash += t_end - t_begin;
+    book_turn(c, 2 + round, t_begin, t_begin, t_begin, t_end);
     c->tree_steps[2 + round] = 0;
     c->tree_cap[2 + round] = (uint8_t)cap_of(c, 2 + round);
     if (const uint32_t ce = c->tree_cap[2 + round]) {
@@ -337,6 +361,7 @@
 }
 bool can_gate(const zk_ctx* c, uint32_t round) { return c->fmt.fold == 1 && !c->fmt.coset && !c->fmt.stop && c->early && c->early_ok && !c->checks && round < c->R && !round_on_host(c, round); }
 int enqueue_gated_fold(zk_ctx* c, uint32_t round) {
+    TurnClock clock{c, &zk_ctx::Turn::launch};
     FoldArgs a;
     int rc = fold_args(c->dom, c->d_layers + c->layer_off[1 + round], c->d_layers + c->layer_off[2 + round], c->L - round, round, 0u, a);
     if (rc) return rc;
@@ -367,8 +392,10 @@
 };
 
 void begin_proof(zk_ctx* c) {
-    c->stage_used = 0; c->n_segs = 0; c->seg_words = 0; c->tail_log = 0; c->tail_have = false;
+    c->stage_used = 0; c->n_segs = 0; c->seg_words = 0; c->tail_log = 0; c->tail_have = false; c->tail_vals = nullptr;
     c->t_wait = c->t_host_hash = c->t_launch = 0;
+    if (c->timing) for (auto& t : c->turn) t = zk_ctx::Turn{};
+    c->turn_of = zk_ctx::kTurnStart;
     memset(c->host_nodes, 0, sizeof c->host_nodes);
     memset(c->host_node_cnt, 0, sizeof c->host_node_cnt);
     memset(c->host_vals, 0, sizeof c->host_vals);
@@ -382,7 +409,7 @@
 int settle_pending(zk_ctx* c) { return c->pending_top ? flush_host_parts(c) : (int)ZK_OK; }
 int last_layer_value(zk_ctx* c, uint32_t* out) {
     const uint32_t* v;
-    if (c->tail_have && c->tail_log == c->log_b) v = c->tail_vals.data();
+    if (c->tail_have && c->tail_log == c->log_b) v = c->tail_vals;
     else {
         HIPCHK(hipMemcpyAsync(c->h_small, c->d_layers + c->layer_off[1 + c->R], c->B * 4, hipMemcpyDeviceToHost, c->stream));
         HIPCHK(hipStreamSynchronize(c->stream));
@@ -453,7 +480,7 @@
     const uint32_t* src = c->d_layers + c->layer_off[layer];
     if (lg <= 10) {
         std::vector<uint32_t> v(m);
-        if (c->tail_have && c->tail_log == lg && layer >= 2) v.assign(c->tail_vals.begin(), c->tail_vals.begin() + m);
+        if (c->tail_have && c->tail_log == lg && layer >= 2) v.assign(c->tail_vals, c->tail_vals + m);
         else {
             HIPCHK(hipMemcpyAsync(v.data(), src, m * 4, hipMemcpyDeviceToHost, c->stream));
             HIPCHK(hipStreamSynchronize(c->stream));
@@ -518,6 +545,7 @@
 }
 
 void commit_tree(zk_ctx* c, Channel& ch, uint32_t tree, const uint8_t root[32]) {
+    TurnClock clock{c, &zk_ctx::Turn::chan};
     if (c->tree_cap[tree]) { ch.commit_bytes(c->cap_digests[tree].data(), c->cap_digests[tree].size()); return; }
     ch.commit_hash(root);
     memcpy(c->info.roots[tree], root, 32);
@@ -557,6 +585,21 @@
         t0 = t;
     }
 };
+
+void print_turns(const zk_ctx* c) {
+    zk_ctx::Turn sum;
+    for (uint32_t i = 0; i < 40; ++i) {
+        const uint32_t id = (i + zk_ctx::kTurnStart) % 40;
+        const zk_ctx::Turn& t = c->turn[id];
+        if (t.wait + t.mail + t.hash + t.book + t.chan + t.launch == 0) continue;
+        if (id == zk_ctx::kTurnStart) fprintf(stderr, "[zk timing]   turn start  : enqueue %6.1f us\n", t.launch);
+        else fprintf(stderr, "[zk timing]   turn tree %2u: wait %7.1f, mailbox read %5.2f, hashing %5.2f, bookkeeping %5.2f, channel %5.2f, enqueue %6.2f us\n",
+                     id, t.wait, t.mail, t.hash, t.book, t.chan, t.launch);
+        sum.wait += t.wait; sum.mail += t.mail; sum.hash += t.hash; sum.book += t.book; sum.chan += t.chan; sum.launch += t.launch;
+    }
+    fprintf(stderr, "[zk timing]   turns, sum : wait %7.1f, mailbox read %5.1f, hashing %5.1f, bookkeeping %5.1f, channel %5.1f, enqueue %6.1f us\n",
+            sum.wait, sum.mail, sum.hash, sum.book, sum.chan, sum.launch);
+}
 
 int prove_finish(zk_ctx* c, Channel& ch, HostLaps& lap) {
     const ProofFormat& f = c->fmt;
@@ -637,7 +680,10 @@
     if ((rc = read_commit(c, 0, root))) return rc;
     commit_tree(c, ch, 0, root);
     uint32_t alpha[3];
-    for (int i = 0; i < 3; ++i) alpha[i] = c->info.alpha_raw[i] = ch.get_u32();
+    {
+        TurnClock clock{c, &zk_ctx::Turn::chan};
+        for (int i = 0; i < 3; ++i) alpha[i] = c->info.alpha_raw[i] = ch.get_u32();
+    }
     if (c->fmt.coset) {
         if ((rc = do_compose(c, alpha)) || (rc = do_merkle(c, 1, true, false, c->fmt.steps(0)))) return rc;
     } else if ((rc = do_compose_commit(c, alpha))) return rc;
@@ -648,7 +694,11 @@
     if (c->fmt.fold > 1 || c->fmt.coset || c->fmt.stop) {
         if ((rc = prove_fold_rounds(c, ch))) return rc;
     } else for (uint32_t r = 0; r < R; ++r) {
-        uint32_t beta = c->info.beta_raw[r] = ch.get_u32();
+        uint32_t beta;
+        {
+            TurnClock clock{c, &zk_ctx::Turn::chan};
+            beta = c->info.beta_raw[r] = ch.get_u32();
+        }
         if (c->gate_pending) {
             release_gated_fold(c, r, beta);
             if (can_gate(c, r + 1) && (rc = enqueue_gated_fold(c, r + 1))) return rc;
@@ -665,6 +715,7 @@
     }
     lap("lde .. last root");
     if (timing) fprintf(stderr, "[zk timing]   of which: waiting for the device %.1f us, host hashing (tops + tail) %.1f us\n", c->t_wait, c->t_host_hash);
+    if (timing) print_turns(c);
     return prove_finish(c, ch, lap);
 }
 
@@ -805,6 +856,10 @@
     if ((rc = dom_make(device, log_n, log_b, shift, tail, c->stream, &c->dom))) return bail(rc);
     c->tail = tail;
     c->hinv_host = invmod(c->dom->h);
+    c->tail_xinv.assign(((size_t)2 << kMaxHostLog) - 1, 0u);
+    for (uint32_t k = 0; k <= kMaxHostLog && k + 1 <= c->L; ++k)
+        host_fold_table(powmod(c->hinv_host, (uint64_t)1 << (c->L - k - 1)), k, c->tail_xinv.data() + (((size_t)1 << k) - 1));
+    c->timing = getenv("ZK_HOST_TIMING") != nullptr;
     c->device_bytes += c->dom->device_bytes;
     size_t off = 0;
     for (uint32_t l = 0; l <= c->R + 1; ++l) {
```

Result: no change. 2.931 billion, median of 6 (+0.4%).
